# nh13/DWGSIM

Measured on AMD Instinct MI355X. Metric: M read-pairs/sec (2x150 bp PE), higher is better.
Workload: dtype u8

## Files before the change

dwgsim_amd/csrc/dw_common.hpp:

```cpp
#pragma once
#include <stdint.h>

#define DW_DEV __device__ __forceinline__
#include <dw_intrin.hpp>
#include <dw_probe.hpp>

namespace dw {

enum : uint32_t {
    D_WALK = 1,
    D_WALK_INSLEN = 2,
    D_WALK_INSBASE = 3,
    D_WALK_SITE = 7,
    D_WALK_SITE_REF = 26,
    D_PAIR = 4,
    D_PLACE = 5,
    D_PLACE_NORM = 6,
    D_BASE0 = 8,
    D_QUAL0 = 10,
    D_FLOW0 = 12,
    D_FLOW_REF = 32,
    D_FLOW_EV = 64,
    D_FLOW_PASS2 = 8,
    D_CALIB = 14,
// ... 51 lines not shown
{
    const U4 b = rng_block<UNIFORM_KEY>(k, dom, idx, att, 0, slot >> 1);
    return (slot & 1) ? u_hi(b) : u_lo(b);
}

DW_DEV uint64_t dbl_bits(double x) { union { double d; uint64_t u; } c; c.d = x; return c.u; }
DW_DEV double bits_dbl(uint64_t u) { union { double d; uint64_t u; } c; c.u = u; return c.d; }


template <bool NORMAL = false>
DW_DEV double det_log(double x)
{
    const double ln2_hi = 6.93147180369123816490e-01, ln2_lo = 1.90821492927058770002e-10,
                 Lg1 = 6.666666666666735130e-01, Lg2 = 3.999999999940941908e-01, Lg3 = 2.857142874366239149e-01,
                 Lg4 = 2.222219843214978396e-01, Lg5 = 1.818357216161805012e-01, Lg6 = 1.531383769920937332e-01,
                 Lg7 = 1.479819860511658591e-01;
    uint64_t b = dbl_bits(x);
    int32_t hx = (int32_t)(b >> 32), k = 0;
    if (!NORMAL && hx < 0x00100000) { x *= 0x1p54; k = -54; b = dbl_bits(x); hx = (int32_t)(b >> 32); }
    k += (hx >> 20) - 1023;
    hx &= 0x000fffff;
    int32_t i = (hx + 0x95f64) & 0x100000;
    x = bits_dbl(((uint64_t)(uint32_t)(hx | (i ^ 0x3ff00000)) << 32) | (b & 0xFFFFFFFFull));
    k += (i >> 20);
    const double f = x - 1.0, dk = (double)k;
    const double s = NORMAL ? div_mid(f, 2.0 + f) : f / (2.0 + f);
    const double z = s * s, w = z * z;
    const double t1 = w * (Lg2 + w * (Lg4 + w * Lg6));
    const double t2 = z * (Lg1 + w * (Lg3 + w * (Lg5 + w * Lg7)));
    const double R = t2 + t1;
    i = (hx - 0x6147a) | (0x6b851 - hx);
    if (i > 0) {
        const double hfsq = 0.5 * f * f;
        return dk * ln2_hi - ((hfsq - (s * (hfsq + R) + dk * ln2_lo)) - f);
    }
    return dk * ln2_hi - ((s * (f - R) - dk * ln2_lo) - f);
}

DW_DEV uint32_t geom_gap(uint32_t w, const uint32_t *lg, uint64_t R, int sR)
{
    const uint64_t X = ((uint64_t)w << 1) | 1ull;
    const int p = 63 - __clzll((long long)X);
    const uint64_t M = X << (63 - p);
    const uint32_t idx = (uint32_t)(M >> 55) & 0xFFu, r16 = (uint32_t)(M >> 39) & 0xFFFFu;
    const uint32_t t0 = lg[idx], t1 = lg[idx + 1];
    const uint32_t f = t0 + (uint32_t)(((uint64_t)(t1 - t0) * r16) >> 16);
    const uint64_t Lu = ((uint64_t)(33 - p) << 56) - ((uint64_t)f << 24);
    const uint64_t G = __umul64hi(Lu, R) >> sR;
    return G > 0x3FFFFFFFull ? 0x3FFFFFFFu : (uint32_t)G;
}

DW_DEV int lane_id() { return (int)(threadIdx.x & 63); }

DW_DEV uint32_t wave_incl_scan(uint32_t v)
{
#pragma unroll
    for (int d = 1; d < 64; d <<= 1) { uint32_t o = __shfl_up(v, d); if (lane_id() >= d) v += o; }
    return v;
}
DW_DEV uint64_t shfl_down_u64(uint64_t v, int d)
{
    uint32_t lo = __shfl_down((uint32_t)v, d), hi = __shfl_down((uint32_t)(v >> 32), d);
    return ((uint64_t)hi << 32) | lo;
}
DW_DEV uint64_t wave_sum_u64(uint64_t v)
{
#pragma unroll
    for (int d = 32; d >= 1; d >>= 1) v += shfl_down_u64(v, d);
    uint32_t lo = __shfl((uint32_t)v, 0), hi = __shfl((uint32_t)(v >> 32), 0);
    return ((uint64_t)hi << 32) | lo;
}
DW_DEV uint32_t wave_sum_u32(uint32_t v)
{
#pragma unroll
    for (int d = 32; d >= 1; d >>= 1) v += __shfl_down(v, d);
    return __shfl(v, 0);
}

constexpr uint64_t ST_AGG = 1ull << 62, ST_PREFIX = 2ull << 62, ST_VAL = (1ull << 62) - 1;

DW_DEV void status_store(uint64_t *p, uint64_t v) { __hip_atomic_store(p, v, __ATOMIC_RELAXED, __HIP_MEMORY_SCOPE_AGENT); }
DW_DEV uint64_t status_load(uint64_t *p) { return __hip_atomic_load(p, __ATOMIC_RELAXED, __HIP_MEMORY_SCOPE_AGENT); }

#ifndef DW_LB_SLEEP
#define DW_LB_SLEEP 2
#endif
#ifndef DW_LB_W
#define DW_LB_W 1
#endif
constexpr int LB_W = DW_LB_W;
DW_DEV uint64_t lookback_excl(uint64_t *status, uint32_t t, uint64_t aggregate, uint64_t base)
{
    const int lane = lane_id();
    if (t == 0) { if (lane == 0) status_store(&status[0], ST_PREFIX | ((base + aggregate) & ST_VAL)); return base; }
    if (lane == 0) status_store(&status[t], ST_AGG | (aggregate & ST_VAL));
    uint64_t excl = 0;
    int64_t k = (int64_t)t - 1;
    for (;;) {
        uint64_t v[LB_W];
#pragma unroll
        for (int w = 0; w < LB_W; ++w) {
            const int64_t idx = k - (int64_t)lane * LB_W - w;
            v[w] = idx >= 0 ? status_load(&status[idx]) : ST_PREFIX;
        }
#pragma unroll
        for (int w = 0; w < LB_W; ++w) {
            const int64_t idx = k - (int64_t)lane * LB_W - w;
            if (probe::off(2048) && (v[w] >> 62) == 0) v[w] = ST_PREFIX;
            while ((v[w] >> 62) == 0) { __builtin_amdgcn_s_sleep(DW_LB_SLEEP); v[w] = status_load(&status[idx]); }
        }
        uint64_t mine = 0; bool have = false;
#pragma unroll
        for (int w = 0; w < LB_W; ++w) { if (!have) mine += v[w] & ST_VAL; have = have || (v[w] >> 62) == 2; }
        const uint64_t pm = __ballot(have);
        const int first = pm ? (__ffsll((unsigned long long)pm) - 1) : 64;
        excl += wave_sum_u64(lane <= first ? mine : 0);
        if (pm) break;
        k -= 64 * LB_W;
    }
    if (lane == 0) status_store(&status[t], ST_PREFIX | ((excl + aggregate) & ST_VAL));
    return excl;
}

}
```

dwgsim_amd/csrc/dw_host.cpp:

```cpp
#include <hip/hip_runtime.h>
#include <math.h>
#include <stdio.h>
#include <stdlib.h>
#include <string.h>
#include <limits.h>
#include <ctype.h>
#include <stdarg.h>
#include <stdint.h>
#include <sys/mman.h>
#include <mutex>
#include <thread>
#include <string>
#include <vector>
#include <algorithm>
#include <array>
#include <stddef.h>
#include <type_traits>
#include "../../include/dwgsim_hip.h"
#include "dw_kernels.hpp"
#include "dw_launch.hpp"
#include "dw_mutin.hpp"
#include "dw_mem.hpp"

using namespace dw;
// ... 831 lines not shown

int dwgsim_hip_set_regions(dwgsim_hip_ctx_t *c, const char *path, const char *const *names, const int64_t *lens, int n_contigs, uint64_t *total_len)
{
    if (!c || !path || n_contigs < 0 || (n_contigs && (!names || !lens))) { if (c) c->err = "bad regions arguments"; return DWGSIM_HIP_ERR_ARG; }
    if (c->prm.amplicons) { c->err = "Error: cannot use a regions BED file (-x) when simulating amplicons (-a)\n"; return DWGSIM_HIP_ERR_ARG; }
    std::vector<ContigName> tab;
    for (int i = 0; i < n_contigs; ++i) tab.push_back(ContigName{names[i], lens[i]});
    std::string err;
    if (!parse_regions(path, tab, c->regions, err)) { c->err = err; c->has_regions = false; return DWGSIM_HIP_ERR_ARG; }
    c->has_regions = true;
    uint64_t tot = 0;
    for (size_t q = 0; q < c->regions.start.size(); ++q) tot += c->regions.end[q] - c->regions.start[q];
    if (total_len) *total_len = tot;
    return DWGSIM_HIP_OK;
}

int64_t dwgsim_hip_contig_region_length(dwgsim_hip_ctx_t *c, uint32_t contig_index, const uint8_t *ascii, int64_t len, int64_t *non_acgt, int64_t *region_bases)
{
    if (non_acgt) *non_acgt = 0;
    if (region_bases) *region_bases = len;
    if (!c || !c->has_regions) return len;
    int64_t m = 0, num_n = 0;
    for (size_t q = 0; q < c->regions.contig.size(); ++q) if (c->regions.contig[q] == contig_index) {
        m += c->regions.end[q] - c->regions.start[q];
        for (int64_t p = c->regions.start[q]; p <= (int64_t)c->regions.end[q]; ++p) { const int ch = (p >= 1 && p - 1 < len) ? ascii[p - 1] : 'N'; if (nt4(ch) >= 4) ++num_n; }
    }
    if (non_acgt) *non_acgt = num_n;
    if (region_bases) *region_bases = m;
    if (m == 0) return DWGSIM_HIP_SKIP_NO_REGION;
    if (0.95 < num_n / (double)m) return DWGSIM_HIP_SKIP_NON_ACGT;
    return m;
}

int dwgsim_hip_contig_set_placement_length(dwgsim_hip_ctx_t *c, int contig, int64_t l)
{
    int k = 0;
    Group *g = get_group(c, contig, &k);
    if (!g || l < 0) { if (c) c->err = "bad placement-length arguments"; return DWGSIM_HIP_ERR_ARG; }
    g->m[(size_t)k].l_place = l;
    return DWGSIM_HIP_OK;
}

int dwgsim_hip_set_mutation_input(dwgsim_hip_ctx_t *c, int type, const char *path, const char *const *names, const int64_t *lens, int n_contigs)
{
    if (!c || !path || type < 0 || type > 2 || n_contigs < 0 || (n_contigs && (!names || !lens))) { if (c) c->err = "bad mutation-input arguments"; return DWGSIM_HIP_ERR_ARG; }
    std::vector<ContigName> tab;
    for (int i = 0; i < n_contigs; ++i) tab.push_back(ContigName{names[i], lens[i]});
    std::string err;
    if (!parse_mutation_input(type, path, tab, c->mutin, err)) { c->err = err; c->has_mutin = false; return DWGSIM_HIP_ERR_ARG; }
    c->has_mutin = true;
    return DWGSIM_HIP_OK;
}

static int mut_debug_verdict(dwgsim_hip_ctx_t *c, const Group &g, uint64_t pre, uint64_t post)
{
    auto member_of = [&](uint64_t v) -> int { const int64_t p = (int64_t)(v >> 8); int k = 0; while (k + 1 < (int)g.m.size() && (int64_t)g.m[(size_t)k + 1].start <= p) ++k; return k; };
    uint64_t v = ~0ull;
    if (pre != ~0ull && post != ~0ull) v = member_of(post) < member_of(pre) ? post : pre;
    else v = pre != ~0ull ? pre : post;
    if (v == ~0ull) return DWGSIM_HIP_OK;
    static const char *what[4] = {"", "(c[0]&0x3) != (c[1]&0x3)", "(c[1]&0x3) != (c[2]&0x3)", "(c[0]&0x3) == (c[1]&0x3) || (c[0]&0x3) == (c[2]&0x3)"};
    const Member &m = g.m[(size_t)member_of(v)];
    char b[256]; snprintf(b, sizeof b, "dwgsim: src/mut.c: mut_debug: Assertion `%s' failed. [%s:%lld]\n", what[v & 3], m.name.c_str(), (long long)(v >> 8) - m.start + 1);
    c->err = b;
    return DWGSIM_HIP_ERR_FAILED;
}

static int ensure_ins(dwgsim_hip_ctx_t *c, Group &g, int h, size_t entries, size_t bases)
{
    GroupMem &M = g.mem;
    const size_t want = sizeof(int32_t) * (entries + entries / 4 + 64);
    for (DevMem *b : {&M.d_ins_pos[h], &M.d_ins_len[h], &M.d_ins_off[h]}) HIPC(c, reserve(c, *b, sizeof(int32_t) * entries, want));
    HIPC(c, reserve(c, M.d_ins_bases[h], bases + 16, bases + bases / 4 + 256 + 16));
    return DWGSIM_HIP_OK;
}

static void make_views(hipStream_t st, const Group &g)
{
    const GroupMem &M = g.mem;
    launch_make_view(st, M.d_cells[0].get(), M.d_cells[1].get(), (int64_t)padded_cells(g) & ~(int64_t)15, g.total, M.d_view[0].get(), M.d_view[1].get(),
                     M.d_summ[0].get<uint16_t>(), M.d_summ[1].get<uint16_t>(), M.d_summ2[0].get<uint16_t>(), M.d_summ2[1].get<uint16_t>());
}

static void dirty_chunks(hipStream_t st, bool restore, const Group &g)
{
    const GroupMem &M = g.mem;
    launch_dirty_chunks(st, restore, M.d_dirty.get<uint32_t>(), dirty_words(padded_cells(g)), g.total, M.d_ref.get(), M.d_refview.get(), M.d_refsumm.get<uint16_t>(), M.d_refsumm2.get<uint16_t>(),
                        M.d_cells[0].get(), M.d_cells[1].get(), M.d_view[0].get(), M.d_view[1].get(), M.d_summ[0].get<uint16_t>(), M.d_summ[1].get<uint16_t>(), M.d_summ2[0].get<uint16_t>(), M.d_summ2[1].get<uint16_t>());
}

static void justify(dwgsim_hip_ctx_t *c, hipStream_t st, const Event *ev, Count n, const ContigDev &cd)
{
    if (c->seq_justify) launch_justify_seq(st, ev, n, cd);
    else launch_justify(st, ev, n, cd, c->w_lo.get<int32_t>(), c->w_sufmin.get<int32_t>(), c->w_bound.get<uint8_t>());
}

static int64_t pack_walk_form(int attempt, bool file_driven, bool slots, int restore, bool dense)
{
    return (int64_t)attempt << 16 | (file_driven ? 1 : 0) << 12 | (slots ? 1 : 0) << 8 | restore << 4 | (dense ? 1 : 0);
}

static int walk_file_driven(dwgsim_hip_ctx_t *c, Group &g)
{
    hipStream_t st = c->walk_stream;
    const GroupMem &M = g.mem;
    WalkCounters *wc = c->d_wcounters.get<WalkCounters>();
    const uint32_t np = g.n_patch, nev = g.n_patch_ev;
    const size_t nev1 = nev ? nev : 1;
    if (np && (ensure(c, c->w_ppos, sizeof(int32_t) * np) || ensure(c, c->w_pcells, sizeof(uint16_t) * np) || ensure(c, c->w_ev, sizeof(Event) * nev1) ||
               ensure(c, c->w_lo, sizeof(int32_t) * nev1) || ensure(c, c->w_sufmin, sizeof(int32_t) * (nev1 + 64)) || ensure(c, c->w_bound, nev1))) return DWGSIM_HIP_ERR_DEVICE;
    c->walk_form = pack_walk_form(g.walk_attempt, true, false, g.walk_reset ? 2 : 0, true);
    HIPC(c, hipEventRecord(M.ev_walk0.get(), st));
    if (g.walk_reset) for (int h = 0; h < 2; ++h) if (const int rc = restore_pristine(c, g, h, R_CELLS, st)) return rc;
    HIPC(c, wc_fill(c, WC_FILE, 0xff, st));
    if (np) {
        HIPC(c, hipMemcpyAsync(c->w_ppos.get(), c->h_ppos.data(), sizeof(int32_t) * np, hipMemcpyHostToDevice, st));
        HIPC(c, hipMemcpyAsync(c->w_pcells.get(), c->h_pcells.data(), sizeof(uint16_t) * np, hipMemcpyHostToDevice, st));
        if (nev) HIPC(c, hipMemcpyAsync(c->w_ev.get(), c->h_pev.data(), sizeof(Event) * nev, hipMemcpyHostToDevice, st));
        launch_apply_patches(st, c->w_ppos.get<int32_t>(), c->w_pcells.get<uint16_t>(), np, M.d_cells[0].get(), M.d_cells[1].get());
        launch_mut_debug(st, M.d_ref.get(), M.d_cells[0].get(), M.d_cells[1].get(), g.total, &wc->mut_debug[0]);
        if (nev) justify(c, st, c->w_ev.get<Event>(), Count{nullptr, nev}, group_dev(g));
        launch_mut_debug(st, M.d_ref.get(), M.d_cells[0].get(), M.d_cells[1].get(), g.total, &wc->mut_debug[1]);
    }
    make_views(st, g);
    g.dirty_all = true;
    HIPC(c, hipGetLastError());
    HIPC(c, wc_fetch(c, M, WC_FILE, st));
    HIPC(c, hipEventRecord(M.ev_walk.get(), st));
    return DWGSIM_HIP_OK;
}

enum class Restore { None, Chunks, All };
struct WalkPlan {
    uint32_t cap; size_t ncap, cap_bases;
    uint32_t nblk;
    bool use_slots; uint32_t nbs, slot_cap; size_t slot_bytes;
    Restore restore;
    bool dense;
};

static WalkPlan walk_plan(const dwgsim_hip_ctx_t *c, const Group &g)
{
    WalkPlan P;
    P.cap = g.walk_cap; P.ncap = P.cap ? P.cap : 1; P.cap_bases = g.walk_cap_bases;
    P.nblk = (uint32_t)((g.total + SCAN_POS_PER_BLOCK - 1) / SCAN_POS_PER_BLOCK);
    P.nbs = site_scan_blocks(g.total);
    const double m = (double)site_scan_block_positions() * (c->prm.mut_rate > 0 ? c->prm.mut_rate : 0.0);
    P.slot_cap = (uint32_t)std::min<double>((double)site_scan_block_positions(), m + 8.0 * sqrt(m + 1.0) + 32.0);
    if (c->site_slot_cap >= 0) P.slot_cap = (uint32_t)std::max<int64_t>(1, c->site_slot_cap);
    P.slot_bytes = (size_t)P.nbs * P.slot_cap * sizeof(int32_t);
    P.use_slots = g.walk_attempt == 0 && c->site_slots != 0 && P.nbs > 0 && (c->site_slots > 0 || P.slot_bytes <= std::max<size_t>((size_t)64 << 20, P.ncap * 16));
    P.restore = g.walk_attempt > 0 || g.dirty_all ? Restore::All : g.dirty_any ? Restore::Chunks : Restore::None;
    P.dense = c->seq_justify || c->dense_view;
    return P;
}

static int walk_reserve(dwgsim_hip_ctx_t *c, Group &g, const WalkPlan &P)
{
    if (ensure(c, c->scratch_status, ((size_t)P.nblk + 2) * sizeof(uint64_t)) ||
        ensure(c, c->w_cand, sizeof(int32_t) * P.ncap) || ensure(c, c->w_ev, sizeof(Event) * P.ncap) ||
        ensure(c, c->w_flags, sizeof(uint4) * (P.ncap + 64)) ||
        ensure(c, c->w_lo, sizeof(int32_t) * P.ncap) || ensure(c, c->w_sufmin, sizeof(int32_t) * (P.ncap + 64)) ||
        ensure(c, c->w_bound, P.ncap)) return DWGSIM_HIP_ERR_DEVICE;
    for (int h = 0; h < 2; ++h) if (const int rc = ensure_ins(c, g, h, P.ncap, P.cap_bases)) return rc;
    if (P.use_slots && (ensure(c, c->w_slots, P.slot_bytes) || ensure(c, c->w_slot_aux, 2 * (size_t)P.nbs * sizeof(uint32_t)))) return DWGSIM_HIP_ERR_DEVICE;
    return DWGSIM_HIP_OK;
}

static int walk_launch(dwgsim_hip_ctx_t *c, Group &g, const WalkPlan &P)
{
    hipStream_t st = c->walk_stream;
    const WalkParams wp = walk_params(c);
    const SegTab seg = seg_tab(g);
    const GroupMem &M = g.mem;
    WalkCounters *wc = c->d_wcounters.get<WalkCounters>();
    int32_t *d_cand = c->w_cand.get<int32_t>(); Event *d_ev = c->w_ev.get<Event>(); uint4 *d_flags = c->w_flags.get<uint4>();
    uint32_t *tot4 = &wc->ins[0].entries;
    const Count nc{&wc->n_cand, P.cap};
    HIPC(c, wc_fill(c, WC_RANDOM, 0, st));
    if (P.use_slots) launch_site_scan_slots(st, M.d_refview.get(), g.total, seg, wp, c->w_slots.get<int32_t>(), P.slot_cap, c->w_slot_aux.get<uint32_t>(), d_cand, P.cap, &wc->n_cand, &wc->slot_over);
    else {
        uint64_t *d_status = c->scratch_status.get<uint64_t>();
        HIPC(c, hipMemsetAsync(d_status, 0, ((size_t)P.nblk + 2) * sizeof(uint64_t), st));
        launch_site_scan_list(st, M.d_refview.get(), g.total, seg, wp, d_status, d_status + P.nblk, d_cand, P.cap, &wc->n_cand);
    }
    launch_events(st, d_cand, nc, M.d_ref.get(), seg, wp, d_ev, &wc->max_del);
    launch_resolve(st, d_ev, nc, &wc->max_del, d_flags, tot4);
    ContigDev cd = group_dev(g);
    cd.tot4 = tot4; cd.cap_bases[0] = (uint32_t)std::min<size_t>(ins_bases_cap(g, 0), 0xFFFFFFFFu); cd.cap_bases[1] = (uint32_t)std::min<size_t>(ins_bases_cap(g, 1), 0xFFFFFFFFu);
    launch_apply(st, d_ev, nc, d_flags, cd, wp);
    justify(c, st, d_ev, nc, cd);
    if (P.dense) {
        make_views(st, g);
        g.dirty_all = true;
    } else {
        launch_mark_dirty(st, d_ev, nc, c->w_lo.get<int32_t>(), M.d_dirty.get<uint32_t>());
        dirty_chunks(st, false, g);
        g.dirty_any = true;
    }
    HIPC(c, hipGetLastError());
    return DWGSIM_HIP_OK;
}

static int walk_random(dwgsim_hip_ctx_t *c, Group &g)
{
    const WalkPlan P = walk_plan(c, g);
    if (const int rc = walk_reserve(c, g, P)) return rc;
    c->walk_form = pack_walk_form(g.walk_attempt, false, P.use_slots, (int)P.restore, P.dense);
    hipStream_t st = c->walk_stream;
    HIPC(c, hipEventRecord(g.mem.ev_walk0.get(), st));
    if (P.restore == Restore::All) { for (int h = 0; h < 2; ++h) if (const int rc = restore_pristine(c, g, h, R_ALL, st)) return rc; }
    else if (P.restore == Restore::Chunks) dirty_chunks(st, true, g);
    if (P.restore != Restore::None) { if (const int rc = clear_dirty(c, g, st)) return rc; g.dirty_all = g.dirty_any = false; }
    if (const int rc = walk_launch(c, g, P)) return rc;
    HIPC(c, wc_fetch(c, g.mem, WC_RANDOM, st));
    HIPC(c, hipEventRecord(g.mem.ev_walk.get(), st));
    return DWGSIM_HIP_OK;
}

static void collect_file_mutations(dwgsim_hip_ctx_t *c, const Group &g, HostIns (&hi)[2])
{
    c->h_ppos.clear(); c->h_pcells.clear(); c->h_pev.clear();
    for (size_t k = 0; k < g.m.size(); ++k) {
        const Member &m = g.m[k];
        for (size_t q = 0; q < m.rc.pos.size(); ++q) {
            c->h_ppos.push_back(m.rc.pos[q] + m.start); c->h_pcells.push_back(m.rc.cells[q]);
            if (m.rc.cells[q] & 0x3030) { Event e; e.pos = m.rc.pos[q] + m.start; e.type = 4; e.hap = 3; e.base = 0; e.live = 1; e.len = 1; e.seg = (uint32_t)k; c->h_pev.push_back(e); }
        }
        for (int h = 0; h < 2; ++h) for (const InsPayload &ip : m.rc.ins[h]) {
            hi[h].pos.push_back(ip.pos + m.start); hi[h].len.push_back((uint32_t)ip.bases.size()); hi[h].off.push_back((uint32_t)hi[h].bases.size());
            hi[h].bases.insert(hi[h].bases.end(), ip.bases.begin(), ip.bases.end());
        }
    }
}

static int upload_ins_tables(dwgsim_hip_ctx_t *c, Group &g, HostIns (&hi)[2])
{
    for (int h = 0; h < 2; ++h) {
        const size_t n = hi[h].pos.size(), nb = hi[h].bases.size();
        g.n_ins[h] = (uint32_t)n; g.n_ins_bases[h] = (uint32_t)nb;
        if (const int rc = ensure_ins(c, g, h, n ? n : 1, nb ? nb : 1)) return rc;
        if (n) for (const InsTable &t : ins_tables(g.mem, h, hi[h])) HIPC(c, hipMemcpy(t.dev, t.host, t.bytes, hipMemcpyHostToDevice));
    }
    return DWGSIM_HIP_OK;
}

static void initial_walk_caps(const dwgsim_hip_ctx_t *c, Group &g)
{
    double mean = 0;
    for (const Member &m : g.m) mean += (double)m.l * c->prm.mut_rate;
    g.walk_cap = (uint32_t)std::min<double>((double)g.total, mean + 8.0 * sqrt(mean + 1.0) + 256.0);
    g.walk_cap_bases = (size_t)g.walk_cap * 8 + 4096;
    if (c->walk_cap >= 0) { g.walk_cap = (uint32_t)c->walk_cap; g.walk_cap_bases = 1; }
}

int dwgsim_hip_mutate_async(dwgsim_hip_ctx_t *c, int contig)
{
    Group *gp = get_group(c, contig);
    if (!gp) return DWGSIM_HIP_ERR_ARG;
    Group &g = *gp;
    if (g.walk_pending) { c->err = "mutate: the group's previous walk was not waited for"; return DWGSIM_HIP_ERR_STATE; }
    for (const Slot &sl : c->slot) if (sl.pending && sl.group == c->handles[(size_t)contig].group) { c->err = "mutate: a batch that reads this group is still in flight (wait for it first)"; return DWGSIM_HIP_ERR_STATE; }
    HIPC(c, hipSetDevice(c->device));
    g.walk_reset = g.mutated;
    for (int h = 0; h < 2; ++h) g.n_ins[h] = g.n_ins_bases[h] = 0;
    g.mutated = true; g.n_cand = 0; g.list_valid = false;
    for (int h = 0; h < 2; ++h) g.hap_text[h].valid = false;
    g.walk_attempt = 0;
    if (g.total == 0) return DWGSIM_HIP_OK;
    if (c->has_mutin) {
        HIPC(c, hipStreamSynchronize(c->walk_stream));
        HostIns hi[2];
        collect_file_mutations(c, g, hi);
        g.n_patch = (uint32_t)c->h_ppos.size(); g.n_patch_ev = (uint32_t)c->h_pev.size();
        g.n_cand = g.n_patch_ev;
        HIPC(c, hipStreamSynchronize(c->walk_stream));
        if (const int rc = upload_ins_tables(c, g, hi)) return rc;
    } else initial_walk_caps(c, g);
    if (const int rc = c->has_mutin ? walk_file_driven(c, g) : walk_random(c, g)) return rc;
    g.walk_pending = true;
    return DWGSIM_HIP_OK;
}

static bool walk_fits(const WalkCounters &w, const Group &g)
{
    return !w.slot_over && w.n_cand <= g.walk_cap && w.ins[0].bases <= ins_bases_cap(g, 0) && w.ins[1].bases <= ins_bases_cap(g, 1);
}

static void exact_walk_caps(const WalkCounters &w, Group &g)
{
    g.walk_cap = (uint32_t)std::min<uint64_t>((uint64_t)g.total, (w.slot_over ? (uint64_t)w.n_cand_true : w.n_cand) + 16);
    g.walk_cap_bases = std::max<size_t>(g.walk_cap_bases, (size_t)std::max(w.ins[0].bases, w.ins[1].bases) * 2 + (size_t)g.walk_cap * 8 + 4096);
}

int dwgsim_hip_mutate_wait(dwgsim_hip_ctx_t *c, int contig)
{
// ... 495 lines not shown
    if (per_range) for (int q = 0; q < n; ++q) per_range[q] = 0;
    Launch L;
    if (const int rc = build_ranges(c, r, n, PLACE_PAIRS, L)) return rc;
    const uint64_t n_pairs = L.n_pairs; const uint32_t n_blocks = L.nblk;
    if (n_pairs == 0) return DWGSIM_HIP_OK;
    Group &g = *L.g;
    HIPC(c, hipSetDevice(c->device));
    hipStream_t st = c->count_stream;
    if (g.walk_pending) { if (const int rc = dwgsim_hip_mutate_wait(c, g.first_handle)) return rc; }
    if (g.mem.ev_walk.get() && g.mutated) HIPC(c, hipStreamWaitEvent(st, g.mem.ev_walk.get(), 0));
    if (const int rc = sim_form(c, L.f)) return rc;
    SimArgs &a = L.a; fill_sim_args(c, g, L.f, a);
    const size_t ns = L.segs.size();
    if (ensure(c, c->place_rand, sizeof(uint32_t) * ((size_t)n_blocks + 1)) || ensure(c, c->place_segs, sizeof(SimSeg) * ns) ||
        ensure(c, c->place_aux, PLACE_LISTS * 16 * sizeof(uint32_t) + sizeof(uint64_t) * ns)) return DWGSIM_HIP_ERR_DEVICE;
    if (sizeof(SimSeg) * ns > c->h_place_segs.cap() || sizeof(uint64_t) * ns > c->h_range_rand.cap()) HIPC(c, hipStreamSynchronize(st));
    HIPC(c, c->h_place_segs.reserve(sizeof(SimSeg) * ns, sizeof(SimSeg) * (ns + 64))); HIPC(c, c->h_range_rand.reserve(sizeof(uint64_t) * ns, sizeof(uint64_t) * (ns + 64)));
    const uint64_t *h_range_rand = c->h_range_rand.get<uint64_t>();
    memcpy(c->h_place_segs.get(), L.segs.data(), sizeof(SimSeg) * ns);
    HIPC(c, hipMemcpyAsync(c->place_segs.get(), c->h_place_segs.get(), sizeof(SimSeg) * ns, hipMemcpyHostToDevice, st));
    a.segs = c->place_segs.get<SimSeg>(); a.n_seg = (int32_t)ns; a.n_blocks = n_blocks; a.n_pairs = n_pairs;
    a.block_rand = c->place_rand.get<uint32_t>(); a.counters = c->pcounters.dev();
    const uint64_t waves = (uint64_t)n_blocks * (PLACE_PAIRS / 64);
    const uint32_t cap_full = (uint32_t)((waves + PLACE_LISTS - 1) / PLACE_LISTS) * 64u;
    uint32_t cap = (uint32_t)std::min<uint64_t>(cap_full, 1024 + n_pairs / PLACE_LISTS / 8);
    if (c->place_cap >= 0 && (uint64_t)c->place_cap < cap) cap = (uint32_t)c->place_cap;
    for (int attempt = 0;; ++attempt) {
        if (ensure(c, c->place_list, sizeof(uint32_t) * (size_t)cap * PLACE_LISTS)) return DWGSIM_HIP_ERR_DEVICE;
        a.place_list = c->place_list.get<uint32_t>(); a.place_list_cap = cap;
        a.place_list_n = c->place_aux.get<uint32_t>(); a.range_rand = reinterpret_cast<uint64_t *>(c->place_aux.get<uint8_t>() + PLACE_LISTS * 16 * sizeof(uint32_t));
        HIPC(c, hipMemsetAsync(c->pcounters.dev(), 0, N_COUNTERS * sizeof(uint64_t), st));
        HIPC(c, hipMemsetAsync(c->place_aux.get(), 0, PLACE_LISTS * 16 * sizeof(uint32_t) + sizeof(uint64_t) * ns, st));
        HIPC(c, hipEventRecord(c->ev_cnt0, st));
        launch_place(st, a);
        HIPC(c, hipEventRecord(c->ev_cnt1, st));
        HIPC(c, hipGetLastError());
        HIPC(c, hipMemcpyAsync(c->pcounters.host(), c->pcounters.dev(), N_COUNTERS * sizeof(uint64_t), hipMemcpyDeviceToHost, st));
        HIPC(c, hipMemcpyAsync(c->h_range_rand.get(), a.range_rand, sizeof(uint64_t) * ns, hipMemcpyDeviceToHost, st));
        HIPC(c, hipStreamSynchronize(st));
        { float ms = 0; if (hipEventElapsedTime(&ms, c->ev_cnt0, c->ev_cnt1) == hipSuccess) c->count_us += 1e3 * ms; else (void)hipGetLastError(); }
        if (!(c->pcounters.host()[2] & 16) || attempt > 0) break;
        cap = cap_full;
    }
    if (c->pcounters.host()[2] & 16) { c->err = "count_random: the list of undecided pairs overflowed twice"; return DWGSIM_HIP_ERR_FAILED; }
    if (c->pcounters.host()[2]) { char b[128]; snprintf(b, sizeof b, "\r[dwgsim_core] failed to generate a read after %d trials\n", MAX_ATTEMPTS + 1); c->err = b; return DWGSIM_HIP_ERR_FAILED; }
    c->place_open = c->pcounters.host()[5];
    uint64_t total = 0;
    for (int q = 0, si = 0; q < n; ++q) if (r[q].n_pairs) { total += h_range_rand[si]; if (per_range) per_range[q] = h_range_rand[si]; ++si; }
    if (n_random) *n_random = total;
    return DWGSIM_HIP_OK;
}

int dwgsim_hip_count_random(dwgsim_hip_ctx_t *c, int contig, uint64_t first_ii, uint64_t n_pairs, uint64_t *n_random)
{
    dwgsim_hip_range_t r; memset(&r, 0, sizeof r); r.contig = contig; r.first_ii = first_ii; r.n_pairs = n_pairs;
    return dwgsim_hip_count_random_ranges(c, &r, 1, n_random, nullptr);
}

int dwgsim_hip_set_fail_carry(dwgsim_hip_ctx_t *c, uint64_t carry)
{
    if (!c) return DWGSIM_HIP_ERR_ARG;
    c->carry_override = carry; c->has_carry_override = true;
    return DWGSIM_HIP_OK;
}

static SimPlan sim_plan(const dwgsim_hip_ctx_t *c, const Launch &L)
{
    const dwgsim_hip_params_t &p = c->prm; const SimForm &f = L.f;
    const uint64_t n_pairs = L.n_pairs; const size_t nblk = L.nblk;
    SimPlan P{};
    const int fixed_max = std::max(L.fixed_max, c->rand_fixed_len);
    for (int j = 0; j < 2; ++j) if (p.length[j] > 0) P.cap[j] = (size_t)n_pairs * (size_t)(1 + fixed_max + 120 + 3 + 2 * (p.data_type == 2 ? f.cap : p.length[j]) + 4);
    int bw_bytes = 0, bw_pairs = 0;
    while (bw_bytes < 63 && (((uint64_t)P.cap[0] | 1ull) >> bw_bytes)) ++bw_bytes;
    while (bw_pairs < 63 && (n_pairs >> bw_pairs)) ++bw_pairs;
    P.lb_shift = bw_bytes; P.too_many = p.data_type != 2 && bw_bytes + bw_pairs > 62;
    P.cap[2] = P.cap[0] + P.cap[1];
    if (!L.a.p.has_bwa) P.cap[0] = P.cap[1] = 0;
    if (!L.a.p.has_bfast) P.cap[2] = 0;
    P.block_rand = sizeof(uint32_t) * nblk;
    if (!f.split) P.status = 4 * sizeof(uint64_t) * nblk;
    else { P.split_state = sizeof(uint32_t) * (size_t)f.lds_words * SIM_THREADS * nblk; P.split_hand = 16 * (size_t)SIM_THREADS * nblk; P.split_agg = 16 * nblk; P.split_pre = 32 * nblk; P.split_chunk = 32 * (nblk / 1024 + 1); }
    P.meta = sizeof(uint32_t) * ((size_t)n_pairs + 8);
    P.fail_summ = ((size_t)((n_pairs + 256ull * 64 - 1) / (256ull * 64)) * 4 + 2) * sizeof(uint64_t);
    P.scratch = f.dt == 2 || (f.dt < 2 && f.nthr == SIM_THREADS_LONG);
    if (P.scratch) {
        const int cu_per_xcd = (c->n_cu >= 64 && c->n_cu % 8 == 0) ? c->n_cu / 8 : c->n_cu;
        const bool ion = p.data_type == 2;
        const int per_cu = sim_blocks_per_cu(f.lds, ion ? 8 : 32);
        P.flow_slots = c->flow_slots > 0 ? c->flow_slots : cu_per_xcd * per_cu;
        if ((uint64_t)P.flow_slots > (uint64_t)nblk) P.flow_slots = (int32_t)nblk;
        if (ion) {
            const size_t slot_bytes = (size_t)flow_words_per_lane(f.lds_words) * (size_t)SIM_THREADS * sizeof(uint32_t);
            const size_t fit = std::max<size_t>(1, ((size_t)4 << 30) / (slot_bytes * 8));
            if ((size_t)P.flow_slots > fit) P.flow_slots = (int32_t)fit;
        }
        const size_t words = (ion ? (size_t)flow_words_per_lane(f.lds_words) * (size_t)SIM_THREADS : (size_t)f.lds_words * (size_t)SIM_THREADS_LONG) * (size_t)P.flow_slots * 8;
        P.flow_scratch = words * sizeof(uint32_t); P.flow_free = sizeof(uint64_t) * (256 + 8 * nblk);
    }
    P.segs = sizeof(SimSeg) * L.segs.size();
    if (c->gzip_on) {
        size_t chunks = 0;
        for (int t = 0; t < 3; ++t) { P.gz_chunks[t] = (size_t)gz_chunks(P.cap[t]); chunks += P.gz_chunks[t]; if (P.cap[t]) P.gz_cap[t] = (size_t)gz_capacity(P.cap[t]); }
        P.gz_status = sizeof(uint64_t) * (chunks ? chunks : 1);
    }
    return P;
}

static int sim_reserve(dwgsim_hip_ctx_t *c, int slot, const SimPlan &P)
{
    Slot &sl = c->slot[slot]; DevMem *out = c->out[slot];
    if (sl.fetch_in_flight) { HIPC(c, hipStreamWaitEvent(c->stream, sl.ev_fetched, 0)); bool grows = false; for (int t = 0; t < 3; ++t) if (P.cap[t] + 64 > out[t].cap()) grows = true; if (grows) HIPC(c, hipEventSynchronize(sl.ev_fetched)); sl.fetch_in_flight = false; }
    for (int t = 0; t < 3; ++t) if (ensure(c, out[t], P.cap[t] + 64)) return DWGSIM_HIP_ERR_DEVICE;
    if (ensure(c, c->block_rand, P.block_rand) || ensure(c, c->status_all, P.status) ||
        ensure(c, c->split_state, P.split_state) || ensure(c, c->split_hand, P.split_hand) || ensure(c, c->split_agg, P.split_agg) || ensure(c, c->split_pre, P.split_pre) || ensure(c, c->split_chunk, P.split_chunk) ||
        ensure(c, c->meta, P.meta) || ensure(c, c->fail_summ, P.fail_summ) || ensure(c, c->flow_scratch, P.flow_scratch) || ensure(c, c->flow_free, P.flow_free) || ensure(c, sl.segs, P.segs)) return DWGSIM_HIP_ERR_DEVICE;
    HIPC(c, sl.h_segs.reserve(P.segs, P.segs + 64 * sizeof(SimSeg)));
    for (int t = 0; t < 3; ++t) if (P.gz_cap[t] && ensure(c, sl.gz_out[t], P.gz_cap[t] + 64)) return DWGSIM_HIP_ERR_DEVICE;
    return ensure(c, sl.gz_status, P.gz_status);
}

static ChainSet sim_chain(dwgsim_hip_ctx_t *c, Slot &sl, const dwgsim_hip_range_t *r, int n, bool set_rand, bool rerun)
{
    if (rerun) return ChainSet{sl.d_rerun_chain.get<uint64_t>(), 1, 1, 0};
    const dwgsim_hip_range_t *r_first = nullptr, *r_last = nullptr;
    for (int q = 0; q < n; ++q) if (r[q].n_pairs) { if (!r_first) r_first = &r[q]; r_last = &r[q]; }
    if (!r_first) { r_first = &r[0]; r_last = &r[n - 1]; }
    const bool continues = c->chain_contig == r_first->contig && c->chain_next_ii == r_first->first_ii && r_first->first_ii != 0;
    const ChainSet ch{c->d_chain.get<uint64_t>(), set_rand ? 1 : 0, (c->has_carry_override || !continues) ? 1 : 0, c->has_carry_override ? c->carry_override : 0};
    c->has_carry_override = false; c->chain_contig = r_last->contig; c->chain_next_ii = r_last->first_ii + r_last->n_pairs;
    if (sl.ranges.data() != r) sl.ranges.assign(r, r + n);
    return ch;
}

static int sim_launch(dwgsim_hip_ctx_t *c, int slot, Launch &L, const SimPlan &P, const ChainSet &ch, uint64_t rand_base, bool rerun)
{
    Slot &sl = c->slot[slot]; SimArgs &a = L.a; const SimForm &f = L.f;
    const uint64_t n_pairs = L.n_pairs; const uint32_t nblk = L.nblk;
    for (int t = 0; t < 3; ++t) sl.out_bytes[t] = sl.gz_bytes[t] = 0;
    sl.n_pairs = n_pairs; sl.empty = n_pairs == 0;
    if (n_pairs == 0) { if (ch.set_rand || ch.set_carry) launch_chain_set(c->stream, ch.words, rand_base, ch.set_rand, ch.carry, ch.set_carry); return DWGSIM_HIP_OK; }
    uint32_t opens = 0; for (const SimSeg &s : L.segs) opens |= s.contig_start;
    memcpy(sl.h_segs.get(), L.segs.data(), P.segs);
    HIPC(c, hipMemcpyAsync(sl.segs.get(), sl.h_segs.get(), P.segs, hipMemcpyHostToDevice, c->stream));
    a.segs = sl.segs.get<SimSeg>(); a.n_seg = (int32_t)L.segs.size(); a.n_blocks = nblk; a.n_pairs = n_pairs; a.chain = ch.words; a.lb_shift = P.lb_shift;
    a.meta = c->meta.get<uint32_t>(); a.block_rand = c->block_rand.get<uint32_t>(); a.counters = sl.counters.dev();
    for (int t = 0; t < 3; ++t) a.out[t] = c->out[slot][t].get<uint8_t>();
    for (int j = 0; j < 4; ++j) a.status[j] = f.split ? nullptr : c->status_all.get<uint64_t>() + (size_t)j * (size_t)nblk;
    if (f.split) { a.split_state = c->split_state.get<uint32_t>(); a.split_hand = c->split_hand.get<uint32_t>(); a.split_agg = c->split_agg.get<uint32_t>(); a.split_pre = c->split_pre.get<uint64_t>(); a.split_chunk = c->split_chunk.get<uint64_t>(); }
    if (P.scratch) { a.flow_scratch = c->flow_scratch.get<uint32_t>(); a.flow_free = c->flow_free.get<uint64_t>(); a.flow_slots = P.flow_slots; }
    sl.group = c->handles[(size_t)L.g->first_handle].group;
    launch_init(c->stream, sl.counters.dev(), (uint32_t)N_COUNTERS, a.status[0], f.split ? 0 : 4 * (uint64_t)nblk, a.flow_free, a.flow_free ? 256 + 8 * (uint64_t)nblk : 0,
                ch.words, rand_base, ch.set_rand, ch.carry, ch.set_carry);
    HIPC(c, hipEventRecord(sl.ev_k0, c->stream));
    c->sim_form = (int64_t)f.nthr << 20 | f.lpp << 16 | f.out << 12 | f.dt << 8 | f.wr << 4 | f.split;
    if (!launch_simulate(c->stream, a, f)) { c->err = "simulate: no k_simulate instance for this form"; return DWGSIM_HIP_ERR_FAILED; }
    HIPC(c, hipEventRecord(sl.ev_k1, c->stream));
    sl.cap_mult = c->flow_cap_mult;
    if (!rerun) launch_failrule(c->stream, a.meta, n_pairs, opens, c->fail_summ.get<uint64_t>(), sl.counters.dev(), c->d_chain.get<uint64_t>());
    if (c->gzip_on) {
        HIPC(c, hipMemsetAsync(sl.gz_status.get(), 0, P.gz_status, c->stream));
        size_t off = 0;
        for (int t = 0; t < 3; ++t) {
            if (P.cap[t] == 0) continue;
            launch_gzip(c->stream, a.out[t], &sl.counters.dev()[4 + t], P.cap[t], sl.gz_out[t].get<uint8_t>(), P.gz_cap[t], sl.gz_status.get<uint64_t>() + off, &sl.counters.dev()[28 + t], &sl.counters.dev()[24 + t], &sl.counters.dev()[2],
                        c->d_crc_table.get<uint32_t>(), c->d_crc_shift.get<uint32_t>());
            off += P.gz_chunks[t];
        }
    }
    HIPC(c, hipEventRecord(sl.ev_end, c->stream));
    HIPC(c, hipGetLastError());
    HIPC(c, hipMemcpyAsync(sl.counters.host(), sl.counters.dev(), N_COUNTERS * sizeof(uint64_t), hipMemcpyDeviceToHost, c->stream));
    HIPC(c, hipEventRecord(sl.ev_done, c->stream));
    sl.pending = true;
    return DWGSIM_HIP_OK;
}

static int sim_enqueue(dwgsim_hip_ctx_t *c, const dwgsim_hip_range_t *r, int n, uint64_t rand_base, int slot, bool rerun)
{
    if (!c || slot < 0 || slot >= DWGSIM_HIP_SLOTS) { if (c) c->err = "bad simulate arguments"; return DWGSIM_HIP_ERR_ARG; }
    if (c->slot[slot].pending) { c->err = "simulate: the slot still holds a batch that was not waited for"; return DWGSIM_HIP_ERR_STATE; }
    Launch L;
    if (const int rc = sim_resolve(c, r, n, L)) return rc;
    HIPC(c, hipSetDevice(c->device));
    const SimPlan P = sim_plan(c, L);
    if (P.too_many) { c->err = "too many pairs in one call"; return DWGSIM_HIP_ERR_ARG; }
    if (L.n_pairs) { if (const int rc = sim_reserve(c, slot, P)) return rc; }
    return sim_launch(c, slot, L, P, sim_chain(c, c->slot[slot], r, n, rand_base != DWGSIM_HIP_RAND_CHAIN, rerun), rand_base, rerun);
}

int dwgsim_hip_simulate_ranges_async(dwgsim_hip_ctx_t *c, const dwgsim_hip_range_t *r, int n, uint64_t rand_base, int slot) { return sim_enqueue(c, r, n, rand_base, slot, false); }

int dwgsim_hip_simulate_async(dwgsim_hip_ctx_t *c, int contig, uint64_t first_ii, uint64_t n_pairs, uint64_t rand_base, int slot)
{
    dwgsim_hip_range_t r; memset(&r, 0, sizeof r); r.contig = contig; r.first_ii = first_ii; r.n_pairs = n_pairs;
    return dwgsim_hip_simulate_ranges_async(c, &r, 1, rand_base, slot);
}

int dwgsim_hip_wait(dwgsim_hip_ctx_t *c, int slot, dwgsim_hip_batch_t *out)
{
    if (!c || slot < 0 || slot >= DWGSIM_HIP_SLOTS) { if (c) c->err = "bad slot"; return DWGSIM_HIP_ERR_ARG; }
    Slot &sl = c->slot[slot];
    if (out) memset(out, 0, sizeof *out);
    if (sl.empty) { sl.pending = false; return DWGSIM_HIP_OK; }
    if (!sl.pending) { c->err = "wait: no batch was enqueued on this slot"; return DWGSIM_HIP_ERR_STATE; }
    HIPC(c, hipSetDevice(c->device));
    HIPC(c, hipEventSynchronize(sl.ev_done));
    sl.pending = false;
    uint64_t *h = sl.counters.host();
    if ((h[2] & 2) && !(h[2] & ~(2ull | 8ull)) && c->prm.data_type == 2) {
        uint64_t keep[8]; for (int q = 0; q < 6; ++q) keep[q] = h[16 + q];
        const uint64_t base = h[22];
        while (h[2] & 2) {
            if (sl.cap_mult >= c->flow_cap_mult) {
                if ((int64_t)flow_base_capacity(c) * (int64_t)c->flow_cap_mult * 2 > (int64_t)FLOW_CAP_MAX) break;
                c->flow_cap_mult *= 2;
            }
            if (const int rc = sim_enqueue(c, sl.ranges.data(), (int)sl.ranges.size(), base, slot, true)) return rc;
            HIPC(c, hipEventSynchronize(sl.ev_done));
            sl.pending = false;
        }
        for (int q = 0; q < 6; ++q) h[16 + q] = keep[q];
    }
    if (h[2] & 4) { c->err = "dwgsim-hip: no fragment placement satisfied the target regions (-x) after 2^20 tries (the reference would not terminate)\n"; return DWGSIM_HIP_ERR_FAILED; }
    if (h[2] & 2) { c->err = "dwgsim-hip: a read outgrew its buffer (or degenerated) in the flow-error model\n"; return DWGSIM_HIP_ERR_FAILED; }
    if ((h[2] & ~8ull) || h[20]) {
        char b[128]; snprintf(b, sizeof b, "\r[dwgsim_core] failed to generate a read after %d trials\n", MAX_ATTEMPTS + 1); c->err = b; return DWGSIM_HIP_ERR_FAILED;
    }
    if (h[2] & 8) { c->err = "dwgsim-hip: the gzip output buffer is too small for this text\n"; return DWGSIM_HIP_ERR_FAILED; }
    for (int t = 0; t < 3; ++t) { sl.out_bytes[t] = h[4 + t]; sl.gz_bytes[t] = h[24 + t]; }
    if (c->phases) {
        uint64_t tot = 0; for (int k = 0; k < 8; ++k) tot += h[8 + k];
        fprintf(stderr, "[phases]");
        for (int k = 0; k < 8; ++k) fprintf(stderr, " p%d=%.1f%%", k, tot ? 100.0 * h[8 + k] / tot : 0.0);
        fprintf(stderr, " (ticks %llu)\n", (unsigned long long)tot);
    }
// ... 220 lines not shown
```

dwgsim_amd/csrc/dw_launch.hpp:

```cpp
#pragma once
#include <hip/hip_runtime.h>
#include "dw_kernels.hpp"

namespace dw {
void launch_pack(hipStream_t st, const uint8_t *ascii, uint8_t *ref, uint8_t *h0, uint8_t *h1, int64_t l);
void launch_site_scan_list(hipStream_t st, const uint8_t *refview, int64_t l, SegTab seg, WalkParams wp, uint64_t *status, uint64_t *ticket, int32_t *out, uint32_t cap, uint64_t *n_out);
uint32_t site_scan_blocks(int64_t l);
uint32_t site_scan_block_positions();
void launch_site_scan_slots(hipStream_t st, const uint8_t *refview, int64_t l, SegTab seg, WalkParams wp, int32_t *slots, uint32_t slot_cap, uint32_t *aux, int32_t *out, uint32_t cap, uint64_t *n_out, uint32_t *over);
void launch_mark_dirty(hipStream_t st, const Event *ev, Count n, const int32_t *lo, uint32_t *dirty);
void launch_dirty_chunks(hipStream_t st, bool restore, const uint32_t *dirty, uint32_t n_words, int64_t l_live, const uint8_t *ref, const uint8_t *refview, const uint16_t *refsumm, const uint16_t *refsumm2,
                         uint8_t *cells0, uint8_t *cells1, uint8_t *view0, uint8_t *view1, uint16_t *summ0, uint16_t *summ1, uint16_t *summ2_0, uint16_t *summ2_1);
void launch_scan_excl(hipStream_t st, uint32_t *data, uint32_t n, uint64_t *total_out);
void launch_compact(hipStream_t st, const uint16_t *mask, const uint32_t *block_base, int32_t *out, int64_t l, uint32_t cap);
void launch_events(hipStream_t st, const int32_t *cand, Count n, const uint8_t *ref, SegTab seg, WalkParams wp, Event *ev, uint32_t *max_del);
void walk_debug_seg_min(uint32_t rows);
void launch_resolve(hipStream_t st, Event *ev, Count n, const uint32_t *max_del, uint4 *flags, uint32_t *tot4);
void launch_apply(hipStream_t st, Event *ev, Count n, const uint4 *flags, ContigDev c, WalkParams wp);
void launch_justify_seq(hipStream_t st, const Event *ev, Count n, ContigDev c);
void launch_justify(hipStream_t st, const Event *ev, Count n, ContigDev c, int32_t *lo, int32_t *sufmin, uint8_t *bound);
void launch_mut_debug(hipStream_t st, const uint8_t *ref, const uint8_t *h0, const uint8_t *h1, int64_t l, uint64_t *verdict);
void launch_make_view(hipStream_t st, const uint8_t *cells0, const uint8_t *cells1, int64_t n_cells, int64_t l_live, uint8_t *view0, uint8_t *view1, uint16_t *summ0, uint16_t *summ1, uint16_t *summ2_0, uint16_t *summ2_1);
void launch_apply_patches(hipStream_t st, const int32_t *pos, const uint16_t *cells, uint32_t n, uint8_t *h0, uint8_t *h1);
void launch_collect_mask(hipStream_t st, const uint8_t *h0, const uint8_t *h1, int64_t l, uint16_t *mask, uint32_t *block_count);
void launch_gather(hipStream_t st, const int32_t *pos, uint32_t n, const uint8_t *ref, const uint8_t *h0, const uint8_t *h1, uint32_t *cells);
void launch_hap_len(hipStream_t st, HapDev h, SegTab seg, int64_t l, uint32_t *block_count);
void launch_hap_write(hipStream_t st, HapDev h, SegTab seg, int64_t l, const uint32_t *block_base, const HapRec *rec, uint32_t n_rec, const uint8_t *pool, uint32_t width, uint8_t *text);
void launch_place(hipStream_t st, const SimArgs &a);
bool launch_simulate(hipStream_t st, const SimArgs &a, const SimForm &f);
void launch_calibrate(hipStream_t st, const CalibArgs &a);
void launch_failrule(hipStream_t st, const uint32_t *meta, uint64_t n_pairs, uint32_t opens_contig, uint64_t *summ, uint64_t *counters, uint64_t *chain);
void launch_chain_set(hipStream_t st, uint64_t *chain, uint64_t rand_base, int set_rand, uint64_t carry, int set_carry);
void launch_init(hipStream_t st, uint64_t *counters, uint32_t n_counters, uint64_t *z0, uint64_t n0, uint64_t *z1, uint64_t n1, uint64_t *chain, uint64_t rand_base, int set_rand, uint64_t carry, int set_carry);
void launch_selftest_lazy(hipStream_t st, int mode, uint32_t first, uint64_t n, double sigma, float qk, float qeps, float qlmin, int qnear1, uint64_t *out);
uint64_t gz_chunks(uint64_t n);
uint64_t gz_capacity(uint64_t n);
void gz_host_tables(uint32_t *crc_table, uint32_t *crc_shift);
void launch_gzip(hipStream_t st, const uint8_t *text, const uint64_t *n_dev, uint64_t text_cap, uint8_t *out, uint64_t out_cap, uint64_t *status, uint64_t *ticket, uint64_t *total, uint64_t *flags,
                 const uint32_t *crc_table, const uint32_t *crc_shift);
void launch_count_byte(hipStream_t st, const uint8_t *text, uint64_t n, uint32_t byte, uint64_t *out);
void launch_selftest_fp64(hipStream_t st, uint32_t seed, uint64_t n, uint64_t *mism);
void launch_selftest_text(hipStream_t st, uint64_t first, uint64_t n, uint64_t stride, uint64_t *out);
void launch_selftest_gap(hipStream_t st, const uint32_t *lg, uint64_t R, int sR, uint32_t first, uint64_t n, uint32_t g_lo, uint32_t g_cnt, uint32_t *chg, uint64_t *out);
}
```

dwgsim_amd/csrc/dw_simulate.hip:

```cpp
#include <algorithm>
#include "dw_read.hpp"
#include "dw_launch.hpp"

#ifndef DW_PART
#define DW_PART -1
#endif
#define DW_HAS(part) (DW_PART == -1 || DW_PART == (part))
#ifndef DW_SIM_WAVES
#define DW_SIM_WAVES 5
#endif
#ifndef DW_SOLID_WAVES
#define DW_SOLID_WAVES 4
#endif
#ifndef DW_SIM_WAVES_BOTH
#define DW_SIM_WAVES_BOTH 4
#endif
#ifndef DW_SIMB_WAVES
#define DW_SIMB_WAVES 6
#endif
#ifndef DW_IONA_WAVES
#define DW_IONA_WAVES 4
#endif
#ifndef DW_IONL_WAVES
#define DW_IONL_WAVES 3
// ... 900 lines not shown
        }
        done += (uint32_t)(i1 - i0);
    }
    const uint32_t s0 = wave_sum_u32(up), s1 = wave_sum_u32(clip), s2 = wave_sum_u32(done);
    if ((threadIdx.x & 63) == 0) {
        if (s0) atomicAdd((unsigned long long *)&out[0], (unsigned long long)s0);
        if (s1) atomicAdd((unsigned long long *)&out[1], (unsigned long long)s1);
        atomicAdd((unsigned long long *)&out[2], (unsigned long long)s2);
    }
}
void launch_selftest_gap(hipStream_t st, const uint32_t *lg, uint64_t R, int sR, uint32_t first, uint64_t n, uint32_t g_lo, uint32_t g_cnt, uint32_t *chg, uint64_t *out)
{
    const uint64_t nb = cdiv(cdiv(n, GAP_RUN), 256);
    hipLaunchKernelGGL(k_selftest_gap, dim3((uint32_t)(nb < (1u << 16) ? (nb ? nb : 1) : (1u << 16))), dim3(256), 0, st, lg, R, sR, first, n, g_lo, g_cnt, chg, out);
}
void launch_selftest_fp64(hipStream_t st, uint32_t seed, uint64_t n, uint64_t *mism)
{
    hipLaunchKernelGGL(k_selftest_fp64, dim3(cdiv(n, 256)), dim3(256), 0, st, seed, n, mism);
}
__global__ void __launch_bounds__(1024) k_split_scan1(SimArgs a)
{
    __shared__ uint32_t sm[3][16];
    const uint32_t t = blockIdx.x * 1024u + threadIdx.x;
    uint4 g = make_uint4(0, 0, 0, 0);
    if (t < a.n_blocks) g = reinterpret_cast<const uint4 *>(a.split_agg)[t];
    const uint32_t v[3] = {g.x, g.y, g.z};
    uint32_t ex[3], tot[3];
    block_excl_scan_n<3>(v, sm, ex, tot);
    if (t < a.n_blocks) { uint64_t *o = a.split_pre + 4 * (size_t)t; o[0] = ex[0]; o[1] = ex[1]; o[2] = ex[2]; }
    if (threadIdx.x == 0) { uint64_t *c = a.split_chunk + 4 * (size_t)blockIdx.x; c[0] = tot[0]; c[1] = tot[1]; c[2] = tot[2]; }
}
__global__ void __launch_bounds__(64) k_split_scan2(SimArgs a, int lpp)
{
    const uint32_t nch = (a.n_blocks + 1023u) / 1024u;
    uint64_t run[3] = {0, 0, 0};
    for (uint32_t base = 0; base < nch; base += 64u) {
        const uint32_t c = base + threadIdx.x;
        uint64_t v[3] = {0, 0, 0};
        if (c < nch) for (int k = 0; k < 3; ++k) v[k] = a.split_chunk[4 * (size_t)c + k];
        uint64_t inc[3];
#pragma unroll
        for (int k = 0; k < 3; ++k) {
            uint64_t x = v[k];
#pragma unroll
            for (int d = 1; d < 64; d <<= 1) { const uint32_t ol = (uint32_t)__shfl_up((int)(uint32_t)x, d), oh = (uint32_t)__shfl_up((int)(uint32_t)(x >> 32), d); if (lane_id() >= d) x += ((uint64_t)oh << 32) | ol; }
            inc[k] = x;
        }
        if (c < nch) for (int k = 0; k < 3; ++k) a.split_chunk[4 * (size_t)c + k] = run[k] + inc[k] - v[k];
        for (int k = 0; k < 3; ++k) { const uint32_t lo = (uint32_t)__shfl((int)(uint32_t)inc[k], 63), hi = (uint32_t)__shfl((int)(uint32_t)(inc[k] >> 32), 63); run[k] += ((uint64_t)hi << 32) | lo; }
    }
    if (threadIdx.x == 0) {
        const uint64_t H = hex_digits_sum(a.chain[0], run[0]), G1 = run[1] + H, G2 = run[2] + (lpp == 2 ? H : 0ull);
        const uint64_t nreads = a.n_pairs * (uint64_t)((a.p.len[1] > 0) ? 2 : 1);
        a.counters[3] = run[0];
        a.counters[4] = a.p.has_bwa ? G1 : 0;
        a.counters[5] = a.p.has_bwa ? G2 : 0;
        a.counters[6] = !a.p.has_bfast ? 0 : G1 + G2 - 2 * nreads;
    }
}

struct FailSeg { uint64_t P, S; uint32_t R, bad; };
DW_DEV FailSeg failseg_join(const FailSeg &a, const FailSeg &b)
{
    FailSeg r;
    r.bad = a.bad | b.bad | ((a.R && a.S + b.P > (uint64_t)MAX_ATTEMPTS) ? 1u : 0u);
    r.P = a.R ? a.P : a.P + b.P;
    r.S = b.R ? b.S : a.S + b.S;
    r.R = a.R | b.R;
    return r;
}
DW_DEV FailSeg failseg_wave_join(FailSeg x, int cnt)
{
    const int lane = lane_id();
#pragma unroll
    for (int d = 1; d < 64; d <<= 1) {
        FailSeg o;
        o.P = ((uint64_t)(uint32_t)__shfl_down((int)(uint32_t)(x.P >> 32), d) << 32) | (uint32_t)__shfl_down((int)(uint32_t)x.P, d);
        o.S = ((uint64_t)(uint32_t)__shfl_down((int)(uint32_t)(x.S >> 32), d) << 32) | (uint32_t)__shfl_down((int)(uint32_t)x.S, d);
        o.R = (uint32_t)__shfl_down((int)x.R, d); o.bad = (uint32_t)__shfl_down((int)x.bad, d);
        if ((lane & (2 * d - 1)) == 0 && lane + d < cnt) x = failseg_join(x, o);
    }
    return x;
}
constexpr int FAIL_PAIRS_PER_THREAD = 64;
__global__ void __launch_bounds__(256) k_failrule_a(const uint32_t *__restrict__ meta, uint64_t n_pairs, const uint64_t *__restrict__ counters, uint64_t *__restrict__ summ)
{
    __shared__ FailSeg seg[4];
    if (counters[1] == 0) return;
    const uint64_t first = ((uint64_t)blockIdx.x * 256 + threadIdx.x) * FAIL_PAIRS_PER_THREAD;
    FailSeg s{0, 0, 0, 0};
    for (int q4 = 0; q4 < FAIL_PAIRS_PER_THREAD && first + q4 < n_pairs; q4 += 4) {
        const uint4 v = *reinterpret_cast<const uint4 *>(meta + first + q4);
        const uint32_t mm[4] = {v.x, v.y, v.z, v.w};
#pragma unroll
        for (int u = 0; u < 4; ++u) {
            if (first + q4 + u >= n_pairs) break;
            const uint32_t m = mm[u];
            if (m & 0x40000000u) s = failseg_join(s, FailSeg{0, 0, 1, 0});
            FailSeg one{m & 0x3fffffffu, 0, (m >> 31) ? 0u : 1u, 0};
            if (!one.R) one.S = one.P;
            s = failseg_join(s, one);
        }
    }
    s = failseg_wave_join(s, 64);
    if ((threadIdx.x & 63) == 0) seg[threadIdx.x >> 6] = s;
    __syncthreads();
    if (threadIdx.x == 0) {
        FailSeg t = seg[0];
        for (int k = 1; k < 4; ++k) t = failseg_join(t, seg[k]);
        summ[4 * (uint64_t)blockIdx.x + 0] = t.P; summ[4 * (uint64_t)blockIdx.x + 1] = t.S;
        summ[4 * (uint64_t)blockIdx.x + 2] = t.R; summ[4 * (uint64_t)blockIdx.x + 3] = t.bad;
    }
}
__global__ void __launch_bounds__(64) k_failrule_b(const uint64_t *__restrict__ summ, uint32_t n_blocks, uint64_t n_pairs, uint32_t opens_contig, uint64_t *__restrict__ counters, uint64_t *__restrict__ chain)
{
    FailSeg t{0, 0, (counters[3] < n_pairs || opens_contig) ? 1u : 0u, 0};
    if (counters[1] != 0) {
        const uint32_t per = (n_blocks + 63) / 64, b0 = threadIdx.x * per, b1 = b0 + per < n_blocks ? b0 + per : n_blocks;
        FailSeg x{0, 0, 0, 0};
        for (uint32_t b = b0; b < b1; ++b) {
            const FailSeg nx{summ[4 * (uint64_t)b], summ[4 * (uint64_t)b + 1], (uint32_t)summ[4 * (uint64_t)b + 2], (uint32_t)summ[4 * (uint64_t)b + 3]};
            x = (b == b0) ? nx : failseg_join(x, nx);
        }
        t = failseg_wave_join(x, per ? (int)((n_blocks + per - 1) / per) : 0);
    }
    if (threadIdx.x == 0) {
        const uint64_t carry = chain[1];
        const FailSeg all = failseg_join(FailSeg{carry, carry, 0, 0}, t);
        counters[16] = t.P; counters[17] = t.S; counters[18] = t.R; counters[19] = t.bad;
        counters[20] = (all.bad || all.P > (uint64_t)MAX_ATTEMPTS || all.S > (uint64_t)MAX_ATTEMPTS) ? 1 : 0;
        counters[21] = all.S;
        chain[1] = all.S;
        counters[22] = chain[0];
        chain[0] += counters[3];
    }
}
void launch_failrule(hipStream_t st, const uint32_t *meta, uint64_t n_pairs, uint32_t opens_contig, uint64_t *summ, uint64_t *counters, uint64_t *chain)
{
    const uint32_t nb = cdiv(n_pairs, 256ull * FAIL_PAIRS_PER_THREAD);
    hipLaunchKernelGGL(k_failrule_a, dim3(nb), dim3(256), 0, st, meta, n_pairs, counters, summ);
    hipLaunchKernelGGL(k_failrule_b, dim3(1), dim3(64), 0, st, summ, nb, n_pairs, opens_contig, counters, chain);
}
__global__ void __launch_bounds__(64) k_chain_set(uint64_t *chain, uint64_t rand_base, int set_rand, uint64_t carry, int set_carry)
{
    if (threadIdx.x != 0) return;
    if (set_rand) chain[0] = rand_base;
    if (set_carry) chain[1] = carry;
}
void launch_chain_set(hipStream_t st, uint64_t *chain, uint64_t rand_base, int set_rand, uint64_t carry, int set_carry)
{
    hipLaunchKernelGGL(k_chain_set, dim3(1), dim3(64), 0, st, chain, rand_base, set_rand, carry, set_carry);
}
__global__ void __launch_bounds__(256) k_launch_init(uint64_t *counters, uint32_t n_counters, uint64_t *z0, uint64_t n0, uint64_t *z1, uint64_t n1, uint64_t *chain, uint64_t rand_base, int set_rand, uint64_t carry, int set_carry)
{
    const uint64_t i = (uint64_t)blockIdx.x * 256 + threadIdx.x, stride = (uint64_t)gridDim.x * 256;
    if (i < n_counters) counters[i] = 0;
    for (uint64_t k = i; k < n0; k += stride) z0[k] = 0;
    for (uint64_t k = i; k < n1; k += stride) z1[k] = 0;
    if (i == 0) { if (set_rand) chain[0] = rand_base; if (set_carry) chain[1] = carry; }
}
void launch_init(hipStream_t st, uint64_t *counters, uint32_t n_counters, uint64_t *z0, uint64_t n0, uint64_t *z1, uint64_t n1, uint64_t *chain, uint64_t rand_base, int set_rand, uint64_t carry, int set_carry)
{
    const uint64_t most = n0 > n1 ? n0 : n1, want = (most + 255) / 256;
    hipLaunchKernelGGL(k_launch_init, dim3((uint32_t)(want < 1 ? 1 : want > 2048 ? 2048 : want)), dim3(256), 0, st, counters, n_counters, z0, n0, z1, n1, chain, rand_base, set_rand, carry, set_carry);
}
__global__ void __launch_bounds__(256) k_count_byte(const uint8_t *__restrict__ text, uint64_t n, uint32_t byte, uint64_t *out)
{
    const uint32_t pat = byte * 0x01010101u;
    uint32_t cnt = 0;
    const uint64_t nvec = n / 16;
    for (uint64_t v = (uint64_t)blockIdx.x * 256 + threadIdx.x; v < nvec; v += (uint64_t)gridDim.x * 256) {
        const uint4 q = reinterpret_cast<const uint4 *>(text)[v];
        const uint32_t w[4] = {q.x ^ pat, q.y ^ pat, q.z ^ pat, q.w ^ pat};
#pragma unroll
        for (int k = 0; k < 4; ++k) cnt += (uint32_t)__popc(~(((w[k] & 0x7F7F7F7Fu) + 0x7F7F7F7Fu) | w[k] | 0x7F7F7F7Fu));
    }
    if (blockIdx.x == 0 && threadIdx.x == 0) for (uint64_t q = nvec * 16; q < n; ++q) cnt += text[q] == byte;
    const uint32_t s = wave_sum_u32(cnt);
    if ((threadIdx.x & 63) == 0 && s) atomicAdd((unsigned long long *)out, (unsigned long long)s);
}
void launch_count_byte(hipStream_t st, const uint8_t *text, uint64_t n, uint32_t byte, uint64_t *out)
{
    hipLaunchKernelGGL(k_count_byte, dim3(4096), dim3(256), 0, st, text, n, byte, out);
}
void launch_place(hipStream_t st, const SimArgs &a)
{
    hipLaunchKernelGGL(k_place, dim3(a.n_blocks), dim3(PLACE_PAIRS), 0, st, a);
    const uint32_t per_list = (uint32_t)std::min<uint64_t>(16, std::max<uint64_t>(1, ((uint64_t)a.place_list_cap + 1023) / 1024));
    hipLaunchKernelGGL(k_place_rest, dim3(PLACE_LISTS * per_list), dim3(128), 0, st, a);
    launch_scan_excl(st, a.block_rand, a.n_blocks, &a.counters[3]);
    hipLaunchKernelGGL(k_range_counts, dim3(cdiv((uint64_t)a.n_seg, 256)), dim3(256), 0, st, a);
}
void launch_split_scan(hipStream_t st, const SimArgs &a, int lpp)
{
    hipLaunchKernelGGL(k_split_scan1, dim3(cdiv(a.n_blocks, 1024)), dim3(1024), 0, st, a);
    hipLaunchKernelGGL(k_split_scan2, dim3(1), dim3(64), 0, st, a, lpp);
}
#endif

#if DW_HAS(4)
__global__ void __launch_bounds__(PAIRS_PER_BLOCK) k_calibrate(CalibArgs a)
{
    DW_DYN_SHARED(uint32_t, dyn_lds);
    __shared__ FlowTables s_ft;
    const int tid = (int)threadIdx.x, nthr = PAIRS_PER_BLOCK;
    if (tid < 64) s_ft.flow[tid] = a.flow[tid];
    __syncthreads();
    fill_flow_tables(s_ft, a.flow_len, tid, nthr, a.flow);
    __syncthreads();
    const uint64_t jj = a.first_read + (uint64_t)blockIdx.x * PAIRS_PER_BLOCK + (uint64_t)tid;
    uint32_t *buf = a.scratch + (size_t)blockIdx.x * ((size_t)a.lds_words * nthr) + tid;
    const int capb = 16 * a.lds_words;
    int32_t n_err = 0; int s_out = 0;
    const bool live = jj < a.n_reads;
    const RngKey key{a.seed, 0u};
    const uint32_t dom = D_CALIB + (uint32_t)a.end;
    if (live) {
        const int h0 = ((capb - a.len) & ~7) >> 3;
        for (int w = 0; w * 8 < a.len; ++w) {
            const U4 q0 = rng_block(key, dom, jj, 0, 0, (uint32_t)(2 * w)), q1 = rng_block(key, dom, jj, 0, 0, (uint32_t)(2 * w + 1));
            const uint32_t rw[8] = {q0.x, q0.y, q0.z, q0.w, q1.x, q1.y, q1.z, q1.w};
            uint32_t pairs = 0;
#pragma unroll
            for (int b = 0; b < 8; ++b) if (w * 8 + b < a.len) pairs |= (rw[b] >> 30) << (2 * b);
            const int h = h0 + w;
            reinterpret_cast<uint16_t *>(buf + (h >> 1) * nthr)[h & 1] = (uint16_t)pairs;
        }
    }
    {
        FlowRng rg; rg.seed = a.seed; rg.contig = 0; rg.dom = dom; rg.att = 1; rg.evt = 0; rg.s = 0; rg.ii = jj; rg.w0 = rg.w1 = rg.w2 = rg.w3 = 0;
        const int so = flow_errors(live, rg, s_ft, a.flow_len, a.thr, a.gap_r, a.gap_s, buf, dyn_lds + tid, nthr, 2 * a.stack_words, a.len, 0, capb, &n_err);
        if (live) { s_out = so; if (s_out < 0) { atomicOr((unsigned long long *)&a.counters[2], 2ull); s_out = 0; n_err = 0; } }
    }
    const uint32_t es = wave_sum_u32((uint32_t)n_err), ls = wave_sum_u32((uint32_t)s_out);
    if ((tid & 63) == 0) { atomicAdd((unsigned long long *)&a.counters[8], (unsigned long long)es); atomicAdd((unsigned long long *)&a.counters[9], (unsigned long long)ls); }
}
void launch_calibrate(hipStream_t st, const CalibArgs &a)
{
    hipLaunchKernelGGL(k_calibrate, dim3(cdiv(std::min(a.chunk_reads, a.n_reads - a.first_read), (uint64_t)PAIRS_PER_BLOCK)), dim3(PAIRS_PER_BLOCK), (size_t)a.stack_words * PAIRS_PER_BLOCK * 4, st, a);
}
#endif

#define DW_SIM_OUTS(X, LPP, DT, NTHR, WR, SPLIT) X(LPP, 1, DT, NTHR, WR, SPLIT) X(LPP, 2, DT, NTHR, WR, SPLIT) X(LPP, 3, DT, NTHR, WR, SPLIT)
#define DW_SIM_PART_1(X)  DW_SIM_OUTS(X, 2, 0, 256, 0, 0) DW_SIM_OUTS(X, 2, 0, 256, 1, 0)
#define DW_SIM_PART_2(X)  DW_SIM_OUTS(X, 1, 0, 256, 0, 0) DW_SIM_OUTS(X, 1, 0, 256, 1, 0)
#define DW_SIM_PART_3(X)  DW_SIM_OUTS(X, 2, 2, 256, 1, 0)
#define DW_SIM_PART_4(X)  DW_SIM_OUTS(X, 1, 2, 256, 1, 0)
// ... 58 lines not shown
```

dwgsim_amd/csrc/dw_walk.hip:

```cpp
#include "dw_device.hpp"
#include "dw_launch.hpp"
#include <stdlib.h>

namespace dw {

__global__ void k_pack(const uint8_t *__restrict__ ascii, uint8_t *__restrict__ ref, uint8_t *__restrict__ h0,
                       uint8_t *__restrict__ h1, int64_t l)
{
    const int64_t nchunk = (l + 15) >> 4;
    for (int64_t ch = (int64_t)blockIdx.x * blockDim.x + threadIdx.x; ch < nchunk; ch += (int64_t)gridDim.x * blockDim.x) {
        const int64_t p0 = ch << 4;
        uint32_t w[4] = {0, 0, 0, 0};
        if (p0 + 16 <= l) {
            const uint4 v = *reinterpret_cast<const uint4 *>(ascii + p0);
            const uint32_t in[4] = {v.x, v.y, v.z, v.w};
#pragma unroll
            for (int q = 0; q < 4; ++q)
#pragma unroll
                for (int b = 0; b < 4; ++b) w[q] |= code_of_ascii((in[q] >> (8 * b)) & 0xff) << (8 * b);
        } else {
            for (int b = 0; b < 16; ++b) { const uint32_t c = (p0 + b < l) ? code_of_ascii(ascii[p0 + b]) : 4u; w[b >> 2] |= c << (8 * (b & 3)); }
        }
        const uint4 o = make_uint4(w[0], w[1], w[2], w[3]);
        *reinterpret_cast<uint4 *>(ref + p0) = o;
// ... 7 lines not shown
struct SiteChain {
    uint32_t m, w0, w1, w2, w3;
    DW_DEV uint32_t gap(RngKey key, uint32_t q, const WalkParams &wp, const uint32_t *lg)
    {
        if ((m & 3u) == 0u) { const U4 b = rng_block<false>(key, D_WALK_SITE, (uint64_t)q, 0, 0, m >> 2); w0 = b.x; w1 = b.y; w2 = b.z; w3 = b.w; }
        const uint32_t k = m & 3u; ++m;
        const uint32_t w = (k & 2u) ? ((k & 1u) ? w3 : w2) : ((k & 1u) ? w1 : w0);
        return wp.mut_thr >= 0x100000000ull ? 0u : geom_gap(w, lg, wp.gap_r, wp.gap_s);
    }
};
template <class F>
DW_DEV uint32_t site_window(const uint8_t *__restrict__ refview, int64_t l_total, const SegTab &seg, const WalkParams &wp, const uint32_t *lg, int64_t g0, F &&f)
{
    if (g0 >= l_total || wp.mut_thr == 0) return 0;
    const uint32_t sk = seg_of(seg, g0);
    const int64_t p0 = g0 - seg.start[sk], l = seg.len[sk];
    if (p0 >= l) return 0;
    const RngKey key{wp.seed, seg.cindex[sk]};
    const uint32_t q = (uint32_t)(p0 >> 8);
    const uint32_t lim = l - p0 < SITE_WINDOW ? (uint32_t)(l - p0) : (uint32_t)SITE_WINDOW;
    SiteChain ch; ch.m = 0; ch.w0 = ch.w1 = ch.w2 = ch.w3 = 0;
    uint32_t n = 0;
    for (uint32_t S = ch.gap(key, q, wp, lg); S < lim; S += 1u + ch.gap(key, q, wp, lg)) {
        const int64_t g = g0 + S;
        const uint32_t nib = (refview[g >> 1] >> (4 * (g & 1))) & 15u;
        if (nib < 4u) { f(g, n); ++n; }
    }
    return n;
}

__global__ void __launch_bounds__(SITE_THREADS) k_site_scan_list(const uint8_t *__restrict__ refview, int64_t l_total, SegTab seg, WalkParams wp, uint64_t *status, uint64_t *ticket,
                                                              int32_t *__restrict__ out, uint32_t cap, uint64_t *n_out, uint32_t n_blocks)
{
    __shared__ uint32_t sm[1][16], s_lg[FLOW_LG_ENTRIES];
    __shared__ uint32_t s_t; __shared__ uint64_t s_base;
    for (int q = (int)threadIdx.x; q < FLOW_LG_ENTRIES; q += SITE_THREADS) s_lg[q] = wp.lg[q];
    if (threadIdx.x == 0) s_t = (uint32_t)atomicAdd((unsigned long long *)ticket, 1ull);
    __syncthreads();
    const uint32_t t = uniform_u32(s_t);
    const int64_t g0 = ((int64_t)t * SITE_THREADS + threadIdx.x) * SITE_WINDOW;
    const uint32_t cnt[1] = {site_window(refview, l_total, seg, wp, s_lg, g0, [](int64_t, uint32_t) {})};
    uint32_t off[1], tot[1];
    block_excl_scan_n<1>(cnt, sm, off, tot);
    if (threadIdx.x < 64) {
        const uint64_t g = lookback_excl(status, t, tot[0], 0);
        if (threadIdx.x == 0) { s_base = g; if (t + 1 == n_blocks) *n_out = g + tot[0]; }
    }
    __syncthreads();
    const uint64_t at0 = s_base + off[0];
    if (cnt[0]) (void)site_window(refview, l_total, seg, wp, s_lg, g0, [&](int64_t g, uint32_t k) { if (at0 + k < cap) out[at0 + k] = (int32_t)g; });
}

__global__ void __launch_bounds__(SITE_THREADS) k_site_scan_slots(const uint8_t *__restrict__ refview, int64_t l_total, SegTab seg, WalkParams wp, int32_t *__restrict__ slots, uint32_t slot_cap,
                                                               uint32_t *__restrict__ slot_cnt)
{
    __shared__ uint32_t sm[1][16], s_lg[FLOW_LG_ENTRIES];
    for (int q = (int)threadIdx.x; q < FLOW_LG_ENTRIES; q += SITE_THREADS) s_lg[q] = wp.lg[q];
    __syncthreads();
    const uint32_t t = blockIdx.x;
    const int64_t g0 = ((int64_t)t * SITE_THREADS + threadIdx.x) * SITE_WINDOW;
    const uint32_t cnt[1] = {site_window(refview, l_total, seg, wp, s_lg, g0, [](int64_t, uint32_t) {})};
    uint32_t off[1], tot[1];
    block_excl_scan_n<1>(cnt, sm, off, tot);
    if (threadIdx.x == 0) slot_cnt[t] = tot[0];
    int32_t *const slot = slots + (size_t)t * slot_cap;
    const uint32_t at0 = off[0];
    if (cnt[0]) (void)site_window(refview, l_total, seg, wp, s_lg, g0, [&](int64_t g, uint32_t k) { if (at0 + k < slot_cap) slot[at0 + k] = (int32_t)g; });
}
__global__ void __launch_bounds__(1024) k_slot_scan(const uint32_t *__restrict__ slot_cnt, uint32_t nb, uint32_t slot_cap, uint32_t *__restrict__ slot_base, uint64_t *n_out, uint32_t *over)
{
    __shared__ uint32_t sm[17];
    __shared__ uint32_t s_over;
    if (threadIdx.x == 0) s_over = 0;
    const uint32_t per = (nb + 1023u) / 1024u, a = threadIdx.x * per, b = a + per < nb ? a + per : nb;
    uint32_t sum = 0; bool big = false;
    for (uint32_t q = a; q < b; ++q) { const uint32_t c = slot_cnt[q]; sum += c; big |= c > slot_cap; }
    uint32_t total;
    uint32_t run = block_excl_scan(sum, sm, &total);
    if (big) atomicOr(&s_over, 1u);
    for (uint32_t q = a; q < b; ++q) { slot_base[q] = run; run += slot_cnt[q]; }
    __syncthreads();
    if (threadIdx.x == 0) { const bool o = s_over != 0; *n_out = o ? 0ull : (uint64_t)total; if (o) { over[0] = 1u; over[1] = total; } }
}
__global__ void __launch_bounds__(256) k_slot_gather(const int32_t *__restrict__ slots, uint32_t slot_cap, const uint32_t *__restrict__ slot_cnt, const uint32_t *__restrict__ slot_base,
                                                     int32_t *__restrict__ out, uint32_t cap)
{
    const uint32_t t = blockIdx.x, base = slot_base[t];
    uint32_t n = slot_cnt[t]; if (n > slot_cap) n = slot_cap;
    for (uint32_t k = threadIdx.x; k < n; k += 256u) if (base + k < cap) out[base + k] = slots[(size_t)t * slot_cap + k];
}

__global__ void k_mark_dirty(const Event *__restrict__ ev, Count nc, const int32_t *__restrict__ lo, uint32_t *__restrict__ dirty)
{
    const uint32_t n = count_of(nc), k = blockIdx.x * blockDim.x + threadIdx.x;
    if (k >= n) return;
    const Event e = ev[k];
    if (!e.live) return;
    const int64_t right = (int64_t)e.pos + (e.type == 2 ? (int64_t)e.len - 1 : 0);
    const int64_t a = (int64_t)(lo[k] < e.pos ? lo[k] : e.pos) >> 6, b = right >> 6;
    for (int64_t q = a; q <= b; ++q) atomicOr(&dirty[q >> 5], 1u << (q & 31));
}
template <bool RESTORE, bool PER_CHUNK>
__global__ void __launch_bounds__(256) k_dirty_chunks(const uint32_t *__restrict__ dirty, uint32_t n_words, int64_t l_live, const uint8_t *__restrict__ ref, const uint8_t *__restrict__ refview,
                                                      const uint16_t *__restrict__ refsumm, const uint16_t *__restrict__ refsumm2,
                                                      uint8_t *__restrict__ cells0, uint8_t *__restrict__ cells1, uint8_t *__restrict__ view0, uint8_t *__restrict__ view1,
                                                      uint16_t *__restrict__ summ0, uint16_t *__restrict__ summ1, uint16_t *__restrict__ summ2_0, uint16_t *__restrict__ summ2_1)
{
    const uint64_t gid = (uint64_t)blockIdx.x * 256u + threadIdx.x;
    const uint32_t w = PER_CHUNK ? (uint32_t)(gid >> 5) : (uint32_t)gid;
    const bool in = w < n_words;
    const uint32_t touched = in ? dirty[w] : 0u;
    if (PER_CHUNK) { if (!__ballot(touched != 0u)) return; }
    else if (!touched) return;
    uint32_t bits = PER_CHUNK ? ((touched >> (gid & 31u)) & 1u) << (gid & 31u) : touched;
    uint32_t fine[2] = {0u, 0u};
    const bool mine = bits != 0u;
    while (bits) {
        const int q = __ffs((int)bits) - 1; bits &= bits - 1;
        const int64_t ch = (int64_t)w * 32 + q, first = ch * SUMM_CELLS;
        if (RESTORE) {
#pragma unroll
            for (int k = 0; k < SUMM_CELLS / 16; ++k) { const uint4 v = *reinterpret_cast<const uint4 *>(ref + first + 16 * k); *reinterpret_cast<uint4 *>(cells0 + first + 16 * k) = v; *reinterpret_cast<uint4 *>(cells1 + first + 16 * k) = v; }
#pragma unroll
            for (int k = 0; k < SUMM_CELLS / 32; ++k) { const uint4 v = *reinterpret_cast<const uint4 *>(refview + (first >> 1) + 16 * k); *reinterpret_cast<uint4 *>(view0 + (first >> 1) + 16 * k) = v; *reinterpret_cast<uint4 *>(view1 + (first >> 1) + 16 * k) = v; }
            const uint16_t sv = refsumm[ch]; summ0[ch] = sv; summ1[ch] = sv;
        } else {
#pragma unroll
            for (int h = 0; h < 2; ++h) {
                const uint8_t *cells = h ? cells1 : cells0; uint8_t *view = h ? view1 : view0;
                uint32_t indel = 0, non_acgt = 0;
#pragma unroll
                for (int half = 0; half < SUMM_CELLS / 32; ++half) {
                    uint32_t out[4] = {0, 0, 0, 0};
#pragma unroll
                    for (int qq = 0; qq < 2; ++qq) {
                        const int64_t at = first + 32 * half + 16 * qq;
                        const uint4 v = *reinterpret_cast<const uint4 *>(cells + at);
                        const uint32_t wd[4] = {v.x, v.y, v.z, v.w};
#pragma unroll
                        for (int b = 0; b < 16; ++b) {
                            const uint32_t c = (wd[b >> 2] >> (8 * (b & 3))) & 0xffu, ty = c & TMASK, base = c & 0xfu;
                            const uint32_t nib = ty == T_NONE ? (base < 4 ? base : base == 4 ? 8u : 9u) : (ty == T_SUB && base < 4) ? 4u + base : 15u;
                            const int cell = 16 * qq + b;
                            out[cell >> 3] |= nib << (4 * (cell & 7));
                        }
#pragma unroll
                        for (int k = 0; k < 4; ++k) {
                            const int64_t rem = l_live - (at + 4 * k);
                            const uint32_t lm = rem >= 4 ? 0xFFFFFFFFu : rem <= 0 ? 0u : ((1u << (8 * (int)rem)) - 1u);
                            indel += (uint32_t)__popc(wd[k] & lm & 0x10101010u);
                            non_acgt |= wd[k] & lm & 0x0C0C0C0Cu;
                        }
                    }
                    *reinterpret_cast<uint4 *>(view + ((first + 32 * half) >> 1)) = make_uint4(out[0], out[1], out[2], out[3]);
                }
                fine[h] = indel | (non_acgt ? 0x8000u : 0u);
                (h ? summ1 : summ0)[ch] = (uint16_t)fine[h];
            }
        }
    }
    static_assert(SUMM2_CELLS / SUMM_CELLS == 16, "a coarse summary = the sixteen lanes of half a bitmap word");
    if (!PER_CHUNK) {
#pragma unroll
        for (int half = 0; half < 2; ++half) {
            if (!((touched >> (16 * half)) & 0xFFFFu)) continue;
            const int64_t s2 = (int64_t)w * 2 + half;
            if (s2 * SUMM2_CELLS >= l_live) continue;
            if (RESTORE) { const uint16_t sv = refsumm2[s2]; summ2_0[s2] = sv; summ2_1[s2] = sv; }
            else {
#pragma unroll
                for (int h = 0; h < 2; ++h) {
                    const uint16_t *sm1 = h ? summ1 : summ0;
                    uint32_t cnt = 0, fl = 0;
                    for (int k = 0; k < SUMM2_CELLS / SUMM_CELLS; ++k) { const int64_t c2 = s2 * (SUMM2_CELLS / SUMM_CELLS) + k; if (c2 * SUMM_CELLS < l_live) { const uint32_t v = sm1[c2]; cnt += v & 0x7fffu; fl |= v & 0x8000u; } }
                    (h ? summ2_1 : summ2_0)[s2] = (uint16_t)(cnt | fl);
                }
            }
        }
        return;
    }
    const int q = (int)(gid & 31u);
    const int64_t ch = (int64_t)w * 32 + q;
    const int64_t s2 = (int64_t)w * 2 + (q >> 4);
    const bool live2 = in && ((touched >> (16 * (q >> 4))) & 0xFFFFu) != 0u && s2 * SUMM2_CELLS < l_live;
    if (RESTORE) { if (live2 && (q & 15) == 0) { const uint16_t sv = refsumm2[s2]; summ2_0[s2] = sv; summ2_1[s2] = sv; } }
    else {
#pragma unroll
        for (int h = 0; h < 2; ++h) {
            uint32_t v = 0;
            if (live2 && ch * SUMM_CELLS < l_live) v = mine ? fine[h] : (uint32_t)(h ? summ1 : summ0)[ch];
            uint32_t cnt = v & 0x7fffu, fl = v & 0x8000u;
#pragma unroll
            for (int m = 1; m < 16; m <<= 1) { cnt += (uint32_t)__shfl_xor((int)cnt, m); fl |= (uint32_t)__shfl_xor((int)fl, m); }
            if (live2 && (q & 15) == 0) (h ? summ2_1 : summ2_0)[s2] = (uint16_t)(cnt | fl);
        }
    }
}

__global__ void k_scan_excl(uint32_t *data, uint32_t n, uint64_t *total_out)
{
    __shared__ uint32_t sm[2][1][16];
    uint64_t grand = 0; int buf = 0;
    for (uint32_t base = 0; base < n; base += blockDim.x, buf ^= 1) {
        const uint32_t i = base + threadIdx.x;
        const uint32_t v[1] = {i < n ? data[i] : 0u};
        uint32_t ex[1], total[1];
        block_excl_scan_n<1>(v, sm[buf], ex, total);
        if (i < n) data[i] = ex[0] + (uint32_t)grand;
        grand += total[0];
    }
    if (total_out && threadIdx.x == 0) *total_out = grand;
}

__global__ void k_compact(const uint16_t *__restrict__ mask, const uint32_t *__restrict__ block_base, int32_t *__restrict__ out, uint32_t cap)
{
    __shared__ uint32_t sm[17];
    uint32_t bits = mask[(int64_t)blockIdx.x * SCAN_THREADS + threadIdx.x];
    uint32_t total;
    uint32_t off = block_base[blockIdx.x] + block_excl_scan((uint32_t)__popc(bits), sm, &total);
    const int64_t p0 = ((int64_t)blockIdx.x * SCAN_THREADS + threadIdx.x) * SCAN_POS_PER_THREAD;
    while (bits) { const int b = __ffs((int)bits) - 1; bits &= bits - 1; if (off < cap) out[off] = (int32_t)(p0 + b); ++off; }
}

__global__ void k_events(const int32_t *__restrict__ cand, Count nc, const uint8_t *__restrict__ ref, SegTab seg,
                         WalkParams wp, Event *__restrict__ ev, uint32_t *__restrict__ max_del)
{
    const uint32_t n_cand = count_of(nc);
    const uint32_t k = blockIdx.x * blockDim.x + threadIdx.x;
    if (k < n_cand) {
        const int64_t g = cand[k];
        const uint32_t sk = seg_of(seg, g);
        const RngKey key{wp.seed, seg.cindex[sk]};
        const int64_t p = g - seg.start[sk], l = seg.len[sk];
        const uint32_t c = ref[g];
        const U4 b1 = rng_block<false>(key, D_WALK, (uint64_t)p, 0, 0, 1);
        const U4 b2 = rng_block<false>(key, D_WALK, (uint64_t)p, 0, 0, 2);
        Event e; e.pos = (int32_t)g; e.live = 1; e.len = 1; e.base = (uint8_t)c; e.seg = sk;
        if (u_lo(b1) >= wp.indel_frac) {
            e.type = 1;
            e.base = (uint8_t)((c + (uint32_t)(uint64_t)(u_hi(b1) * 3.0 + 1)) & 3);
            e.hap = (wp.is_hap || u_lo(b2) < 0.333333) ? 3 : (u_hi(b2) < 0.5 ? 1 : 2);
        } else if (u_hi(b1) < 0.5) {
            e.type = 2;
            e.hap = (wp.is_hap || u_lo(b2) < 0.3333333) ? 3 : (u_hi(b2) < 0.5 ? 1 : 2);
            uint32_t len = 1;
            for (int64_t q = p + 1; q < l; ++q) {
                if ((int64_t)len < wp.indel_min || rng_slot<false>(key, D_WALK, (uint64_t)q, 0, 0) < wp.indel_extend) ++len; else break;
            }
            e.len = len;
            atomicMax(max_del, len);
        } else {
            e.type = 3;
            uint64_t num = 0; uint32_t kk = 0;
            do { ++num; } while (num < 0xFFFFFFFFull && ((int64_t)num < wp.indel_min || rng_slot<false>(key, D_WALK_INSLEN, (uint64_t)p, 0, kk++) < wp.indel_extend));
            e.len = (uint32_t)num;
            e.hap = (wp.is_hap || u_lo(b2) < 0.333333) ? 3 : (u_hi(b2) < 0.5 ? 1 : 2);
        }
        ev[k] = e;
    }
}

DW_DEV bool reached_by_any(const Event *ev, uint32_t k, uint32_t max_del)
{
    const int64_t pk = ev[k].pos;
    for (int64_t j = (int64_t)k - 1; j >= 0; --j) {
        const int64_t pj = ev[j].pos;
        if (pk - pj >= (int64_t)max_del) break;
        if (ev[j].type == 2 && pj + (int64_t)ev[j].len - 1 >= pk) return true;
    }
    return false;
}
__global__ void k_resolve(Event *ev, Count nc, const uint32_t *max_del_p, uint4 *flags)
{
    const uint32_t n_cand = count_of(nc);
    const uint32_t k = blockIdx.x * blockDim.x + threadIdx.x;
    if (k >= n_cand) return;
    const uint32_t max_del = *max_del_p;
    bool live = true;
    if (max_del > 1 && reached_by_any(ev, k, max_del)) {
        int64_t a = (int64_t)k - 1;
        while (a > 0 && reached_by_any(ev, (uint32_t)a, max_del)) --a;
        int64_t reach = -1;
        for (int64_t m = a; m <= (int64_t)k; ++m) {
            const bool lv = ev[m].pos > reach;
            if (lv && ev[m].type == 2) reach = (int64_t)ev[m].pos + ev[m].len - 1;
            live = lv;
        }
    }
    const Event e = ev[k];
    uint4 f;
    f.x = (live && e.type == 3 && (e.hap & 1)) ? 1u : 0u;
    f.y = (live && e.type == 3 && (e.hap & 1)) ? e.len : 0u;
    f.z = (live && e.type == 3 && (e.hap & 2)) ? 1u : 0u;
    f.w = (live && e.type == 3 && (e.hap & 2)) ? e.len : 0u;
    if (!live) f.x |= 0x80000000u;
    flags[k] = f;
}

constexpr uint32_t WALK_SEGS = 32;
static uint32_t g_walk_seg_min_rows = 16384;
void walk_debug_seg_min(uint32_t rows) { g_walk_seg_min_rows = rows ? rows : 16384; }
__global__ void k_scan4(uint4 *flags, Count nc, uint32_t *tot, uint32_t seglen, uint4 *part)
{
    const uint32_t n = count_of(nc);
    const uint32_t lo = seglen ? blockIdx.x * seglen : 0u, hi = seglen ? (lo + seglen < n ? lo + seglen : n) : n;
    constexpr uint32_t ITEMS = 8;
    __shared__ uint32_t sm[2][4][16];
    uint32_t c0 = 0, c1 = 0, c2 = 0, c3 = 0; int buf = 0;
    for (uint32_t base = lo; base < hi; base += blockDim.x * ITEMS, buf ^= 1) {
        const uint32_t i0 = base + threadIdx.x * ITEMS;
        uint4 v[ITEMS];
#pragma unroll
        for (uint32_t q = 0; q < ITEMS; ++q) v[q] = i0 + q < hi ? flags[i0 + q] : make_uint4(0, 0, 0, 0);
        uint32_t t[4] = {0, 0, 0, 0};
#pragma unroll
        for (uint32_t q = 0; q < ITEMS; ++q) {
            const uint32_t dead = v[q].x & 0x80000000u, x = v[q].x & 0x7fffffffu, y = v[q].y, z = v[q].z, w = v[q].w;
            v[q] = make_uint4(t[0] | dead, t[1], t[2], t[3]);
            t[0] += x; t[1] += y; t[2] += z; t[3] += w;
        }
        uint32_t ex[4], total[4];
        block_excl_scan_n<4>(t, sm[buf], ex, total);
#pragma unroll
        for (uint32_t q = 0; q < ITEMS; ++q)
            if (i0 + q < hi) flags[i0 + q] = make_uint4(((v[q].x & 0x7fffffffu) + ex[0] + c0) | (v[q].x & 0x80000000u), v[q].y + ex[1] + c1, v[q].z + ex[2] + c2, v[q].w + ex[3] + c3);
        c0 += total[0]; c1 += total[1]; c2 += total[2]; c3 += total[3];
    }
    if (threadIdx.x == 0) { if (seglen) part[blockIdx.x] = make_uint4(c0, c1, c2, c3); else { tot[0] = c0; tot[1] = c1; tot[2] = c2; tot[3] = c3; } }
}
__global__ void k_scan4_fix(uint4 *flags, Count nc, uint32_t *tot, uint32_t seglen, const uint4 *part)
{
    const uint32_t n = count_of(nc), i = blockIdx.x * blockDim.x + threadIdx.x, s = i / seglen;
    uint32_t a0 = 0, a1 = 0, a2 = 0, a3 = 0, t0 = 0, t1 = 0, t2 = 0, t3 = 0;
    for (uint32_t q = 0; q < WALK_SEGS; ++q) { const uint4 p = part[q]; if (q < s) { a0 += p.x; a1 += p.y; a2 += p.z; a3 += p.w; } t0 += p.x; t1 += p.y; t2 += p.z; t3 += p.w; }
    if (i == 0) { tot[0] = t0; tot[1] = t1; tot[2] = t2; tot[3] = t3; }
    if (i < n && s) { const uint4 f = flags[i]; flags[i] = make_uint4(((f.x & 0x7fffffffu) + a0) | (f.x & 0x80000000u), f.y + a1, f.z + a2, f.w + a3); }
}

__global__ void k_apply(Event *ev, Count nc, const uint4 *flags, ContigDev c, WalkParams wp)
{
    const uint32_t n_cand = count_of(nc);
    adopt_device_sizes(c);
    if (c.tot4 && (c.tot4[1] > c.cap_bases[0] || c.tot4[3] > c.cap_bases[1])) return;
    const uint32_t k = blockIdx.x * blockDim.x + threadIdx.x;
    if (k >= n_cand) return;
    const uint4 f = flags[k];
    Event e = ev[k];
    if (f.x & 0x80000000u) { ev[k].live = 0; return; }
    const int64_t p = e.pos;
    if (e.type == 1) {
        if (e.hap & 1) c.hap[0].cells[p] = T_SUB | e.base;
        if (e.hap & 2) c.hap[1].cells[p] = T_SUB | e.base;
    } else if (e.type == 2) {
        for (uint32_t q = 0; q < e.len; ++q) {
            const uint8_t v = T_DEL | c.ref[p + q];
            if (e.hap & 1) c.hap[0].cells[p + q] = v;
            if (e.hap & 2) c.hap[1].cells[p + q] = v;
        }
    } else {
        const RngKey key{wp.seed, c.seg.cindex[e.seg]};
        const uint64_t pl = (uint64_t)(p - c.seg.start[e.seg]);
        const uint32_t idx[2] = {f.x & 0x7fffffffu, f.z}, off[2] = {f.y, f.w};
        for (int h = 0; h < 2; ++h) if (e.hap & (1 << h)) {
            c.hap[h].cells[p] = T_INS | e.base;
            c.hap[h].ins_pos[idx[h]] = (int32_t)p;
            c.hap[h].ins_len[idx[h]] = e.len;
            c.hap[h].ins_off[idx[h]] = off[h];
        }
        for (uint32_t j = 0; j < e.len; ++j) {
            const uint8_t b = (uint8_t)(uint64_t)(rng_slot<false>(key, D_WALK_INSBASE, pl, 0, j) * 4.0);
            if (e.hap & 1) c.hap[0].ins_bases[off[0] + e.len - 1 - j] = b;
            if (e.hap & 2) c.hap[1].ins_bases[off[1] + e.len - 1 - j] = b;
        }
    }
}

DW_DEV void justify_ins(HapDev &h, int64_t i, int64_t lo)
{
    const uint32_t idx = ins_find(h, i);
    const uint32_t n = h.ins_len[idx];
    uint8_t *P = h.ins_bases + h.ins_off[idx];
    int64_t j = i;
    while (j > lo && (h.cells[j - 1] & TMASK) == T_NONE && P[n - 1] == (h.cells[j - 1] & 3)) {
        for (uint32_t t = n - 1; t > 0; --t) P[t] = P[t - 1];
        P[0] = h.cells[j - 1] & 3;
        h.cells[j] = h.cells[j] & 3;
        --j;
    }
    h.cells[j] = T_INS | (h.cells[j] & 3);
    h.ins_pos[idx] = (int32_t)j;
}
DW_DEV void del_swap(HapDev &h, int64_t j, int64_t dl)
{
    const uint8_t t = h.cells[j]; h.cells[j] = h.cells[j + dl]; h.cells[j + dl] = (uint8_t)((t | TMASK) ^ TMASK);
}
DW_DEV int64_t del_run(const HapDev &h, int64_t i, int64_t l)
{
    int64_t dl = 1;
    for (int64_t j = i + 1; j < l && (h.cells[j] & TMASK) == T_DEL; ++j) ++dl;
    return dl;
}
DW_DEV void justify_visit(ContigDev &c, int64_t i, int *prev_del, int64_t lo, int64_t hi)
{
    if (c.ref[i] >= 4) return;
    HapDev &h0 = c.hap[0], &h1 = c.hap[1];
    const uint8_t c1 = h0.cells[i], c2 = h1.cells[i];
    if ((c1 & TMASK) == T_NONE && (c2 & TMASK) == T_NONE) { prev_del[0] = prev_del[1] = 0; return; }
    if ((c1 & BTMASK) == (c2 & BTMASK)) {
        if ((c1 & TMASK) == T_SUB) { prev_del[0] = prev_del[1] = 0; }
        else if ((c1 & TMASK) == T_DEL) {
            if (prev_del[0] == 1 || prev_del[1] == 1) return;
            prev_del[0] = prev_del[1] = 1;
            const int64_t dl = del_run(h0, i, hi);
            if (hi <= i + dl) return;
            if (i > lo) for (int64_t j = i - 1;; --j) {
                const uint8_t a = h0.cells[j], b = h1.cells[j];
                if ((a & TMASK) != T_INS && (b & TMASK) != T_INS && (a & TMASK) != T_DEL && (b & TMASK) != T_DEL
                    && (a & 3) == (h0.cells[j + dl] & 3) && (b & 3) == (h1.cells[j + dl] & 3)) { del_swap(h0, j, dl); del_swap(h1, j, dl); }
                else break;
                if (j == lo) break;
            }
        } else { prev_del[0] = prev_del[1] = 0; justify_ins(h0, i, lo); justify_ins(h1, i, lo); }
    } else {
        if ((c1 & TMASK) == T_SUB || (c2 & TMASK) == T_SUB) { prev_del[0] = prev_del[1] = 0; }
        else if ((c1 & TMASK) == T_DEL || (c2 & TMASK) == T_DEL) {
            const int x = ((c1 & TMASK) == T_DEL) ? 0 : 1;
            if (prev_del[x] == 1) return;
            prev_del[x] = 1;
            HapDev &h = c.hap[x];
            const int64_t dl = del_run(h, i, hi);
            if (hi <= i + dl) return;
            if (i > lo) for (int64_t j = i - 1;; --j) {
                const uint8_t a = h.cells[j];
                if ((a & TMASK) == T_NONE && (a & 3) == (h.cells[j + dl] & 3)) del_swap(h, j, dl); else break;
                if (j == lo) break;
            }
        } else if ((c1 & TMASK) == T_INS) { prev_del[0] = prev_del[1] = 0; justify_ins(h0, i, lo); }
        else { prev_del[0] = prev_del[1] = 0; justify_ins(h1, i, lo); }
    }
}
__global__ void k_justify_seq(const Event *ev, Count nc, ContigDev c)
{
    const uint32_t n_cand = count_of(nc);
    adopt_device_sizes(c);
    if (blockIdx.x != 0 || threadIdx.x != 0) return;
    int prev_del[2] = {0, 0};
    int64_t last = -1; uint32_t cur = 0xFFFFFFFFu;
    for (uint32_t k = 0; k < n_cand; ++k) {
        const Event e = ev[k];
        if (!e.live) continue;
        const int64_t lo = c.seg.start[e.seg], hi = lo + c.seg.len[e.seg];
        if (e.seg != cur) { cur = e.seg; prev_del[0] = prev_del[1] = 0; last = lo - 1; }
        const int64_t p = e.pos, right = p + (e.type == 2 ? (int64_t)e.len - 1 : 0);
        if (prev_del[0] | prev_del[1])
            for (int64_t q = last + 1; q < p; ++q) if (c.ref[q] < 4) { prev_del[0] = prev_del[1] = 0; break; }
        for (int64_t i = p; i <= right; ++i) justify_visit(c, i, prev_del, lo, hi);
        last = right;
    }
}

DW_DEV int64_t reach_del(const ContigDev &c, int h, int64_t p, int64_t lo, int64_t hi)
{
    const int64_t L = del_run(c.hap[h], p, hi);
    const uint8_t *cl = c.hap[h].cells;
    int64_t j = p - 1;
    for (; j >= lo; --j) {
        const bool mutated = ((c.hap[0].cells[j] | c.hap[1].cells[j]) & TMASK) != 0;
        if (!(mutated || (p + L < hi && (cl[j] & 3) == (cl[j + L] & 3)))) break;
    }
    return j < lo ? lo : j;
}
DW_DEV int64_t reach_ins(const ContigDev &c, int h, int64_t p, int64_t lo)
{
    const uint32_t idx = ins_find(c.hap[h], p);
    const uint32_t n = c.hap[h].ins_len[idx];
    const uint8_t *P = c.hap[h].ins_bases + c.hap[h].ins_off[idx];
    int64_t j = p - 1; int64_t r = 0;
    for (; j >= lo; --j, ++r) {
        const bool mutated = ((c.hap[0].cells[j] | c.hap[1].cells[j]) & TMASK) != 0;
        const uint32_t last = r < (int64_t)n ? (uint32_t)P[n - 1 - r] : (uint32_t)(c.ref[p - 1 - (r - n)] & 3);
        if (!(mutated || last == (uint32_t)(c.ref[j] & 3))) break;
    }
    return j < lo ? lo : j;
}
__global__ void k_jreach(const Event *__restrict__ ev, Count nc, ContigDev c, int32_t *__restrict__ lo)
{
    const uint32_t n_cand = count_of(nc);
    adopt_device_sizes(c);
    const uint32_t k = blockIdx.x * blockDim.x + threadIdx.x;
    if (k >= n_cand) return;
    const Event e = ev[k];
    int64_t reach = 0x7fffffff;
    if (e.live) {
        const int64_t p = e.pos, lo = c.seg.start[e.seg], hi = lo + c.seg.len[e.seg];
        reach = p;
        if (e.type == 2) reach = reach_del(c, (e.hap & 1) ? 0 : 1, p, lo, hi);
        else if (e.type == 3) reach = reach_ins(c, (e.hap & 1) ? 0 : 1, p, lo);
        else if (e.type == 4) {
            for (int h = 0; h < 2; ++h) {
                const uint8_t t = c.hap[h].cells[p] & TMASK;
                int64_t r = p;
                if (t == T_DEL) r = reach_del(c, h, p, lo, hi); else if (t == T_INS) r = reach_ins(c, h, p, lo);
                if (r < reach) reach = r;
            }
        }
    }
    lo[k] = (int32_t)reach;
}
__global__ void k_sufmin(const int32_t *__restrict__ lo, Count nc, int32_t *__restrict__ sufmin, uint32_t seglen, int32_t *part)
{
    const uint32_t n = count_of(nc);
    const int64_t a = seglen ? (int64_t)blockIdx.x * seglen : 0, b = seglen ? (a + seglen < (int64_t)n ? a + seglen : (int64_t)n) : (int64_t)n;
    __shared__ int32_t sm[2][16];
    int32_t carry = 0x7fffffff; int buf = 0;
    const int lane = lane_id(), wave = (int)(threadIdx.x >> 6), nw = (int)(blockDim.x >> 6);
    const uint32_t nchunk = b > a ? (uint32_t)((b - a + blockDim.x - 1) / blockDim.x) : 0u;
    for (uint32_t ch = 0; ch < nchunk; ++ch, buf ^= 1) {
        const int64_t i = b - 1 - ((int64_t)ch * blockDim.x + threadIdx.x);
        int32_t v = i >= a ? lo[i] : 0x7fffffff;
#pragma unroll
        for (int d = 1; d < 64; d <<= 1) { const int32_t o = __shfl_up(v, d); if (lane >= d && o < v) v = o; }
        if (lane == 63) sm[buf][wave] = v;
        __syncthreads();
        int32_t pre = carry, all = carry;
        for (int w = 0; w < nw; ++w) { const int32_t t = sm[buf][w]; if (t < all) all = t; if (w < wave && t < pre) pre = t; }
        if (pre < v) v = pre;
        if (i >= a) sufmin[i] = v;
        carry = all;
    }
    if (seglen && threadIdx.x == 0) part[blockIdx.x] = carry;
}
__global__ void k_sufmin_fix(int32_t *__restrict__ sufmin, Count nc, uint32_t seglen, const int32_t *__restrict__ part)
{
    const uint32_t n = count_of(nc), i = blockIdx.x * blockDim.x + threadIdx.x, s = i / seglen;
    int32_t m = 0x7fffffff;
    for (uint32_t q = 0; q < WALK_SEGS; ++q) { const int32_t p = part[q]; if (q > s && p < m) m = p; }
    if (i < n && m < sufmin[i]) sufmin[i] = m;
}
__global__ void k_jbound(const Event *__restrict__ ev, Count nc, ContigDev c, const int32_t *__restrict__ sufmin, uint8_t *__restrict__ bound)
{
    const uint32_t n_cand = count_of(nc);
    adopt_device_sizes(c);
    const uint32_t k = blockIdx.x * blockDim.x + threadIdx.x;
    if (k >= n_cand) return;
    uint8_t b = 0;
    if (ev[k].live) {
        int64_t a = (int64_t)k - 1;
        while (a >= 0 && !ev[a].live) --a;
        if (a < 0 || ev[a].seg != ev[k].seg) b = 1;
        else {
            const int64_t right_a = (int64_t)ev[a].pos + (ev[a].type == 2 ? (int64_t)ev[a].len - 1 : 0);
            if ((int64_t)sufmin[k] > right_a) {
                for (int64_t q = right_a + 1; q < (int64_t)ev[k].pos; ++q) if (c.ref[q] < 4) { b = 1; break; }
            }
        }
    }
    bound[k] = b;
}
__global__ void k_jrun(const Event *__restrict__ ev, Count nc, ContigDev c, const uint8_t *__restrict__ bound)
{
    const uint32_t n_cand = count_of(nc);
    adopt_device_sizes(c);
    const uint32_t k0 = blockIdx.x * blockDim.x + threadIdx.x;
    if (k0 >= n_cand || !bound[k0]) return;
    int prev_del[2] = {0, 0};
    int64_t last = -1;
    for (uint32_t k = k0; k < n_cand; ++k) {
        const Event e = ev[k];
        if (!e.live) continue;
        if (k > k0 && bound[k]) break;
        const int64_t p = e.pos, right = p + (e.type == 2 ? (int64_t)e.len - 1 : 0);
        const int64_t lo = c.seg.start[e.seg], hi = lo + c.seg.len[e.seg];
        if (k > k0 && (prev_del[0] | prev_del[1]))
            for (int64_t q = last + 1; q < p; ++q) if (c.ref[q] < 4) { prev_del[0] = prev_del[1] = 0; break; }
        for (int64_t i = p; i <= right; ++i) justify_visit(c, i, prev_del, lo, hi);
        last = right;
    }
}

__global__ void k_apply_patches(const int32_t *__restrict__ pos, const uint16_t *__restrict__ cells, uint32_t n, uint8_t *h0, uint8_t *h1)
{
    const uint32_t k = blockIdx.x * blockDim.x + threadIdx.x;
    if (k < n) { h0[pos[k]] = (uint8_t)(cells[k] & 0xff); h1[pos[k]] = (uint8_t)(cells[k] >> 8); }
}

__global__ void k_collect_mask(const uint8_t *__restrict__ h0, const uint8_t *__restrict__ h1, int64_t l,
                               uint16_t *__restrict__ mask, uint32_t *__restrict__ block_count)
{
    __shared__ uint32_t sm[17];
    const int64_t p0 = ((int64_t)blockIdx.x * SCAN_THREADS + threadIdx.x) * SCAN_POS_PER_THREAD;
    uint32_t bits = 0;
    if (p0 < l) {
        const uint4 a = *reinterpret_cast<const uint4 *>(h0 + p0), b = *reinterpret_cast<const uint4 *>(h1 + p0);
        const uint32_t m[4] = {(a.x | b.x) & 0x30303030u, (a.y | b.y) & 0x30303030u, (a.z | b.z) & 0x30303030u, (a.w | b.w) & 0x30303030u};
#pragma unroll
        for (int q = 0; q < 16; ++q) if (((m[q >> 2] >> (8 * (q & 3))) & 0xff) && p0 + q < l) bits |= 1u << q;
    }
    mask[(int64_t)blockIdx.x * SCAN_THREADS + threadIdx.x] = (uint16_t)bits;
    uint32_t total;
    (void)block_excl_scan((uint32_t)__popc(bits), sm, &total);
    if (threadIdx.x == 0) block_count[blockIdx.x] = total;
}
__global__ void k_gather(const int32_t *__restrict__ pos, uint32_t n, const uint8_t *__restrict__ ref, const uint8_t *__restrict__ h0, const uint8_t *__restrict__ h1, uint32_t *__restrict__ cells)
{
    const uint32_t k = blockIdx.x * blockDim.x + threadIdx.x;
    if (k < n) { const int32_t p = pos[k]; cells[k] = (uint32_t)h0[p] | ((uint32_t)h1[p] << 8) | ((uint32_t)ref[p] << 16) | ((uint32_t)(p > 0 ? ref[p - 1] : 4) << 24); }
}

DW_DEV uint32_t hap_char(uint32_t code) { return code < 4u ? (0x54474341u >> (8u * code)) & 0xffu : (uint32_t)'N'; }
DW_DEV uint32_t hap_cell(const uint4 &v, int q) { const uint32_t w = (q & 8) ? ((q & 4) ? v.w : v.z) : ((q & 4) ? v.y : v.x); return (w >> (8 * (q & 3))) & 0xffu; }
DW_DEV uint32_t hap_ins_entry(const HapDev &h, int64_t g)
{
    const uint32_t idx = ins_find(h, g);
    return idx < h.n_ins && (int64_t)h.ins_pos[idx] == g ? idx : h.n_ins;
}
DW_DEV uint32_t hap_emitted(const HapDev &h, int64_t g, const uint4 &v, int nv)
{
    if (((v.x | v.y | v.z | v.w) & 0x10101010u) == 0) return (uint32_t)nv;
    uint32_t n = 0;
    for (int q = 0; q < nv; ++q) {
        const uint32_t ty = hap_cell(v, q) & TMASK;
        if (ty == T_DEL) continue;
        ++n;
        if (ty == T_INS) { const uint32_t idx = hap_ins_entry(h, g + q); if (idx < h.n_ins) n += h.ins_len[idx]; }
    }
    return n;
}
__global__ void __launch_bounds__(SCAN_THREADS) k_hap_len(HapDev h, SegTab seg, uint32_t *__restrict__ block_count)
{
    __shared__ uint32_t sm[17];
    const int64_t g0 = (int64_t)blockIdx.x * SCAN_POS_PER_BLOCK, g = g0 + (int64_t)threadIdx.x * SCAN_POS_PER_THREAD;
    const uint32_t sk = seg_of(seg, g0);
    const int64_t end = (int64_t)seg.start[sk] + seg.len[sk];
    uint32_t cnt = 0;
    if (g < end) { const uint4 v = *reinterpret_cast<const uint4 *>(h.cells + g); cnt = hap_emitted(h, g, v, end - g < 16 ? (int)(end - g) : 16); }
// ... 18 lines not shown
    const int64_t end = (int64_t)seg.start[sk] + seg.len[sk];
    uint4 v = make_uint4(0, 0, 0, 0); int nv = 0; uint32_t cnt = 0;
    if (g < end) { v = *reinterpret_cast<const uint4 *>(h.cells + g); nv = end - g < 16 ? (int)(end - g) : 16; cnt = hap_emitted(h, g, v, nv); }
    uint32_t total;
    const uint32_t off = block_excl_scan(cnt, sm, &total);
    if (total == 0) return;
    const HapRec R = rec[sk];
    const uint32_t B = block_base[blockIdx.x] - R.base0, len = R.n_bases;
    const uint64_t body = R.rec_off + R.hdr_len;
    const uint64_t body_bytes = (uint64_t)len + (width ? ((uint64_t)len + width - 1) / width : 1u);
    const bool plain = ((v.x | v.y | v.z | v.w) & 0x10101010u) == 0;
    for (uint32_t w0 = 0; w0 < total; w0 += HAP_WINDOW) {
        const uint32_t nb = total - w0 < (uint32_t)HAP_WINDOW ? total - w0 : (uint32_t)HAP_WINDOW;
        if (w0) __syncthreads();
        if (cnt && off < w0 + nb && off + cnt > w0) {
            uint32_t e = off;
            auto put = [&](uint32_t code) { if (e >= w0 && e - w0 < nb) stage[e - w0] = (uint8_t)hap_char(code); ++e; };
            for (int q = 0; q < nv; ++q) {
                const uint32_t c = hap_cell(v, q), ty = c & TMASK;
                if (ty == T_DEL) continue;
                put(c & 0xfu);
                if (!plain && ty == T_INS) {
                    const uint32_t idx = hap_ins_entry(h, g + q);
                    if (idx < h.n_ins) { const uint32_t n = h.ins_len[idx]; const uint8_t *P = h.ins_bases + h.ins_off[idx]; for (uint32_t j = 0; j < n; ++j) put(P[j]); }
                }
            }
        }
        __syncthreads();
        const uint32_t b0 = B + w0, b1 = b0 + nb;
        const uint32_t r0 = width ? b0 % width : 0u;
        const uint64_t aS = body + b0 + (width ? b0 / width : 0u);
        const uint64_t aE = body + (b1 == len ? body_bytes : (uint64_t)b1 + (width ? b1 / width : 0u));
        for (uint64_t wa = (aS & ~(uint64_t)15) + 16u * (uint64_t)threadIdx.x; wa < aE; wa += 16u * (uint64_t)SCAN_THREADS) {
            const int first = wa < aS ? (int)(aS - wa) : 0;
            const uint32_t d = (uint32_t)(wa + (uint64_t)first - aS), x = r0 + d;
            uint32_t line = 0, col = x;
            if (width) { line = x / (width + 1u); col = x - line * (width + 1u); }
            uint32_t bl = line * width + col - r0;
            uint32_t out[4] = {0, 0, 0, 0};
#pragma unroll
            for (int i = 0; i < 16; ++i) {
                if (i < first || wa + (uint64_t)i >= aE) continue;
                const bool nl = width && col == width;
                const uint32_t ch = (nl || bl >= nb) ? (uint32_t)'\n' : (uint32_t)stage[bl];
                if (nl) col = 0; else { ++col; ++bl; }
                out[i >> 2] |= ch << (8 * (i & 3));
            }
            if (first == 0 && wa + 16u <= aE) *reinterpret_cast<uint4 *>(text + wa) = make_uint4(out[0], out[1], out[2], out[3]);
            else {
#pragma unroll
                for (int i = 0; i < 16; ++i) if (i >= first && wa + (uint64_t)i < aE) text[wa + (uint64_t)i] = (uint8_t)(out[i >> 2] >> (8 * (i & 3)));
            }
        }
    }
}

void launch_hap_len(hipStream_t st, HapDev h, SegTab seg, int64_t l, uint32_t *block_count)
{
    if (l > 0) hipLaunchKernelGGL(k_hap_len, dim3(cdiv((uint64_t)l, SCAN_POS_PER_BLOCK)), dim3(SCAN_THREADS), 0, st, h, seg, block_count);
}
void launch_hap_write(hipStream_t st, HapDev h, SegTab seg, int64_t l, const uint32_t *block_base, const HapRec *rec, uint32_t n_rec, const uint8_t *pool, uint32_t width, uint8_t *text)
{
    if (n_rec) hipLaunchKernelGGL(k_hap_headers, dim3(n_rec < 4096u ? n_rec : 4096u), dim3(64), 0, st, rec, n_rec, pool, text);
    if (l > 0) hipLaunchKernelGGL(k_hap_write, dim3(cdiv((uint64_t)l, SCAN_POS_PER_BLOCK)), dim3(SCAN_THREADS), 0, st, h, seg, block_base, rec, width, text);
}
void launch_pack(hipStream_t st, const uint8_t *ascii, uint8_t *ref, uint8_t *h0, uint8_t *h1, int64_t l)
{
    const uint64_t nchunk = (uint64_t)(l + 15) >> 4;
    uint32_t nb = cdiv(nchunk, 256); if (nb > (1u << 16)) nb = 1u << 16; if (nb == 0) nb = 1;
    hipLaunchKernelGGL(k_pack, dim3(nb), dim3(256), 0, st, ascii, ref, h0, h1, l);
}
void launch_site_scan_list(hipStream_t st, const uint8_t *refview, int64_t l, SegTab seg, WalkParams wp, uint64_t *status, uint64_t *ticket, int32_t *out, uint32_t cap, uint64_t *n_out)
{
    const uint32_t nb = (uint32_t)cdiv((uint64_t)l, (uint64_t)SITE_BLOCK_POS);
    hipLaunchKernelGGL(k_site_scan_list, dim3(nb), dim3(SITE_THREADS), 0, st, refview, l, seg, wp, status, ticket, out, cap, n_out, nb);
}
uint32_t site_scan_blocks(int64_t l) { return (uint32_t)cdiv((uint64_t)l, (uint64_t)SITE_BLOCK_POS); }
uint32_t site_scan_block_positions() { return (uint32_t)SITE_BLOCK_POS; }
void launch_site_scan_slots(hipStream_t st, const uint8_t *refview, int64_t l, SegTab seg, WalkParams wp, int32_t *slots, uint32_t slot_cap, uint32_t *aux, int32_t *out, uint32_t cap, uint64_t *n_out, uint32_t *over)
{
    const uint32_t nb = site_scan_blocks(l);
    if (!nb) return;
    hipLaunchKernelGGL(k_site_scan_slots, dim3(nb), dim3(SITE_THREADS), 0, st, refview, l, seg, wp, slots, slot_cap, aux);
    hipLaunchKernelGGL(k_slot_scan, dim3(1), dim3(1024), 0, st, aux, nb, slot_cap, aux + nb, n_out, over);
    hipLaunchKernelGGL(k_slot_gather, dim3(nb), dim3(256), 0, st, slots, slot_cap, aux, aux + nb, out, cap);
}
void launch_mark_dirty(hipStream_t st, const Event *ev, Count n, const int32_t *lo, uint32_t *dirty)
{
    if (n.host) hipLaunchKernelGGL(k_mark_dirty, dim3(cdiv(n.host, 256)), dim3(256), 0, st, ev, n, lo, dirty);
}
void launch_dirty_chunks(hipStream_t st, bool restore, const uint32_t *dirty, uint32_t n_words, int64_t l_live, const uint8_t *ref, const uint8_t *refview, const uint16_t *refsumm, const uint16_t *refsumm2,
                         uint8_t *cells0, uint8_t *cells1, uint8_t *view0, uint8_t *view1, uint16_t *summ0, uint16_t *summ1, uint16_t *summ2_0, uint16_t *summ2_1)
{
    if (!n_words) return;
    bool per_chunk = (uint64_t)n_words * 32 <= (1ull << 21);
    if (const char *e = getenv("DWGSIM_HIP_DIRTY_MAP")) per_chunk = e[0] == 'c';
    const dim3 grid(cdiv((uint64_t)n_words * (per_chunk ? 32 : 1), 256));
    if (restore) { if (per_chunk) hipLaunchKernelGGL((k_dirty_chunks<true, true>), grid, dim3(256), 0, st, dirty, n_words, l_live, ref, refview, refsumm, refsumm2, cells0, cells1, view0, view1, summ0, summ1, summ2_0, summ2_1); else hipLaunchKernelGGL((k_dirty_chunks<true, false>), grid, dim3(256), 0, st, dirty, n_words, l_live, ref, refview, refsumm, refsumm2, cells0, cells1, view0, view1, summ0, summ1, summ2_0, summ2_1); }
    else { if (per_chunk) hipLaunchKernelGGL((k_dirty_chunks<false, true>), grid, dim3(256), 0, st, dirty, n_words, l_live, ref, refview, refsumm, refsumm2, cells0, cells1, view0, view1, summ0, summ1, summ2_0, summ2_1); else hipLaunchKernelGGL((k_dirty_chunks<false, false>), grid, dim3(256), 0, st, dirty, n_words, l_live, ref, refview, refsumm, refsumm2, cells0, cells1, view0, view1, summ0, summ1, summ2_0, summ2_1); }
}
void launch_scan_excl(hipStream_t st, uint32_t *data, uint32_t n, uint64_t *total_out)
{
    hipLaunchKernelGGL(k_scan_excl, dim3(1), dim3(1024), 0, st, data, n, total_out);
}
void launch_compact(hipStream_t st, const uint16_t *mask, const uint32_t *block_base, int32_t *out, int64_t l, uint32_t cap)
{
    hipLaunchKernelGGL(k_compact, dim3(cdiv((uint64_t)l, SCAN_POS_PER_BLOCK)), dim3(SCAN_THREADS), 0, st, mask, block_base, out, cap);
}
void launch_events(hipStream_t st, const int32_t *cand, Count n, const uint8_t *ref, SegTab seg, WalkParams wp, Event *ev, uint32_t *max_del)
{
    if (n.host) hipLaunchKernelGGL(k_events, dim3(cdiv(n.host, 256)), dim3(256), 0, st, cand, n, ref, seg, wp, ev, max_del);
}
void launch_resolve(hipStream_t st, Event *ev, Count n, const uint32_t *max_del, uint4 *flags, uint32_t *tot4)
{
    if (n.host) hipLaunchKernelGGL(k_resolve, dim3(cdiv(n.host, 256)), dim3(256), 0, st, ev, n, max_del, flags);
    if (n.host < g_walk_seg_min_rows) { hipLaunchKernelGGL(k_scan4, dim3(1), dim3(1024), 0, st, flags, n, tot4, 0u, (uint4 *)nullptr); return; }
    const uint32_t seglen = (n.host + WALK_SEGS - 1) / WALK_SEGS;
    hipLaunchKernelGGL(k_scan4, dim3(WALK_SEGS), dim3(1024), 0, st, flags, n, tot4, seglen, flags + n.host);
    hipLaunchKernelGGL(k_scan4_fix, dim3(cdiv(n.host, 256)), dim3(256), 0, st, flags, n, tot4, seglen, (const uint4 *)(flags + n.host));
}
void launch_apply(hipStream_t st, Event *ev, Count n, const uint4 *flags, ContigDev c, WalkParams wp)
{
    if (n.host) hipLaunchKernelGGL(k_apply, dim3(cdiv(n.host, 256)), dim3(256), 0, st, ev, n, flags, c, wp);
}
void launch_justify_seq(hipStream_t st, const Event *ev, Count n, ContigDev c)
{
    if (n.host) hipLaunchKernelGGL(k_justify_seq, dim3(1), dim3(64), 0, st, ev, n, c);
}
void launch_justify(hipStream_t st, const Event *ev, Count n, ContigDev c, int32_t *lo, int32_t *sufmin, uint8_t *bound)
{
    if (!n.host) return;
    hipLaunchKernelGGL(k_jreach, dim3(cdiv(n.host, 256)), dim3(256), 0, st, ev, n, c, lo);
    if (n.host < g_walk_seg_min_rows) hipLaunchKernelGGL(k_sufmin, dim3(1), dim3(1024), 0, st, lo, n, sufmin, 0u, (int32_t *)nullptr);
    else {
        const uint32_t seglen = (n.host + WALK_SEGS - 1) / WALK_SEGS;
        hipLaunchKernelGGL(k_sufmin, dim3(WALK_SEGS), dim3(1024), 0, st, lo, n, sufmin, seglen, sufmin + n.host);
        hipLaunchKernelGGL(k_sufmin_fix, dim3(cdiv(n.host, 256)), dim3(256), 0, st, sufmin, n, seglen, (const int32_t *)(sufmin + n.host));
    }
    hipLaunchKernelGGL(k_jbound, dim3(cdiv(n.host, 256)), dim3(256), 0, st, ev, n, c, sufmin, bound);
    hipLaunchKernelGGL(k_jrun, dim3(cdiv(n.host, 64)), dim3(64), 0, st, ev, n, c, bound);
}
__global__ void __launch_bounds__(SCAN_THREADS) k_mut_debug(const uint8_t *__restrict__ ref, const uint8_t *__restrict__ h0, const uint8_t *__restrict__ h1, int64_t l, uint64_t *verdict)
{
    const int64_t first = ((int64_t)blockIdx.x * SCAN_THREADS + threadIdx.x) * SCAN_POS_PER_THREAD;
    if (first >= l) return;
    const uint4 a = *reinterpret_cast<const uint4 *>(h0 + first), b = *reinterpret_cast<const uint4 *>(h1 + first);
    if ((((a.x | a.y | a.z | a.w) | (b.x | b.y | b.z | b.w)) & 0x30303030u) == 0) return;
    const uint4 r = *reinterpret_cast<const uint4 *>(ref + first);
    const uint32_t aw[4] = {a.x, a.y, a.z, a.w}, bw[4] = {b.x, b.y, b.z, b.w}, rw[4] = {r.x, r.y, r.z, r.w};
    for (int q = 0; q < SCAN_POS_PER_THREAD && first + q < l; ++q) {
        const uint32_t c0 = (rw[q >> 2] >> (8 * (q & 3))) & 0xffu, c1 = (aw[q >> 2] >> (8 * (q & 3))) & 0xffu, c2 = (bw[q >> 2] >> (8 * (q & 3))) & 0xffu;
        if (c0 >= 4 || ((c1 & TMASK) == T_NONE && (c2 & TMASK) == T_NONE)) continue;
        uint32_t code = 0;
        if ((c1 & BTMASK) == (c2 & BTMASK)) { if ((c1 & TMASK) == T_SUB && (c0 & 3) == (c1 & 3)) code = 1; }
        else if ((c1 & TMASK) == T_SUB || (c2 & TMASK) == T_SUB) {
            if ((c1 & 3) == (c2 & 3)) code = 2;
            else if (!((c0 & 3) == (c1 & 3) || (c0 & 3) == (c2 & 3))) code = 3;
        }
        if (code) { atomicMin((unsigned long long *)verdict, ((unsigned long long)(first + q) << 8) | code); return; }
    }
}
void launch_mut_debug(hipStream_t st, const uint8_t *ref, const uint8_t *h0, const uint8_t *h1, int64_t l, uint64_t *verdict)
{
    if (l > 0) hipLaunchKernelGGL(k_mut_debug, dim3(cdiv((uint64_t)l, SCAN_POS_PER_BLOCK)), dim3(SCAN_THREADS), 0, st, ref, h0, h1, l, verdict);
}
__global__ void __launch_bounds__(256) k_make_view(const uint8_t *__restrict__ cells0, const uint8_t *__restrict__ cells1, int64_t n_cells, int64_t l_live, uint8_t *__restrict__ view0, uint8_t *__restrict__ view1,
                                                   uint16_t *__restrict__ summ0, uint16_t *__restrict__ summ1, uint16_t *__restrict__ summ2_0, uint16_t *__restrict__ summ2_1)
{
    const uint8_t *__restrict__ cells = blockIdx.y ? cells1 : cells0;
    uint8_t *__restrict__ view = blockIdx.y ? view1 : view0;
    uint16_t *__restrict__ summ = blockIdx.y ? summ1 : summ0, *__restrict__ summ2 = blockIdx.y ? summ2_1 : summ2_0;
    const int64_t t = (int64_t)blockIdx.x * 256 + threadIdx.x, first = t * 32;
    const bool live = first < n_cells;
    uint32_t out[4] = {0, 0, 0, 0}, indel = 0, non_acgt = 0;
    if (live) {
#pragma unroll
        for (int q = 0; q < 2; ++q) {
            if (first + 16 * q >= n_cells) break;
            const uint4 v = *reinterpret_cast<const uint4 *>(cells + first + 16 * q);
            const uint32_t w[4] = {v.x, v.y, v.z, v.w};
#pragma unroll
            for (int b = 0; b < 16; ++b) {
                const uint32_t c = (w[b >> 2] >> (8 * (b & 3))) & 0xffu, ty = c & TMASK, base = c & 0xfu;
                const uint32_t nib = ty == T_NONE ? (base < 4 ? base : base == 4 ? 8u : 9u) : (ty == T_SUB && base < 4) ? 4u + base : 15u;
                const int cell = 16 * q + b;
                out[cell >> 3] |= nib << (4 * (cell & 7));
            }
#pragma unroll
            for (int k = 0; k < 4; ++k) {
                const int64_t rem = l_live - (first + 16 * q + 4 * k);
                const uint32_t lm = rem >= 4 ? 0xFFFFFFFFu : rem <= 0 ? 0u : ((1u << (8 * (int)rem)) - 1u);
                indel += (uint32_t)__popc(w[k] & lm & 0x10101010u);
                non_acgt |= w[k] & lm & 0x0C0C0C0Cu;
            }
        }
        *reinterpret_cast<uint4 *>(view + (first >> 1)) = make_uint4(out[0], out[1], out[2], out[3]);
    }
    uint32_t i1 = indel, f1 = non_acgt ? 1u : 0u;
#pragma unroll
    for (int d = 1; d < SUMM_CELLS / 32; d <<= 1) { i1 += (uint32_t)__shfl_xor((int)i1, d); f1 |= (uint32_t)__shfl_xor((int)f1, d); }
    uint32_t i2 = i1, f2 = f1;
#pragma unroll
    for (int d = SUMM_CELLS / 32; d < SUMM2_CELLS / 32; d <<= 1) { i2 += (uint32_t)__shfl_xor((int)i2, d); f2 |= (uint32_t)__shfl_xor((int)f2, d); }
    if (first < l_live) {
        if ((t & (SUMM_CELLS / 32 - 1)) == 0) summ[t / (SUMM_CELLS / 32)] = (uint16_t)(i1 | (f1 ? 0x8000u : 0u));
        if ((t & (SUMM2_CELLS / 32 - 1)) == 0) summ2[t / (SUMM2_CELLS / 32)] = (uint16_t)(i2 | (f2 ? 0x8000u : 0u));
    }
}
void launch_make_view(hipStream_t st, const uint8_t *cells0, const uint8_t *cells1, int64_t n_cells, int64_t l_live, uint8_t *view0, uint8_t *view1, uint16_t *summ0, uint16_t *summ1, uint16_t *summ2_0, uint16_t *summ2_1)
{
    if (n_cells > 0) hipLaunchKernelGGL(k_make_view, dim3(cdiv((uint64_t)n_cells, 256 * 32), 2), dim3(256), 0, st, cells0, cells1, n_cells, l_live, view0, view1, summ0, summ1, summ2_0, summ2_1);
}
void launch_apply_patches(hipStream_t st, const int32_t *pos, const uint16_t *cells, uint32_t n, uint8_t *h0, uint8_t *h1)
{
    if (n) hipLaunchKernelGGL(k_apply_patches, dim3(cdiv(n, 256)), dim3(256), 0, st, pos, cells, n, h0, h1);
}
void launch_collect_mask(hipStream_t st, const uint8_t *h0, const uint8_t *h1, int64_t l, uint16_t *mask, uint32_t *block_count)
{
    hipLaunchKernelGGL(k_collect_mask, dim3(cdiv((uint64_t)l, SCAN_POS_PER_BLOCK)), dim3(SCAN_THREADS), 0, st, h0, h1, l, mask, block_count);
}
void launch_gather(hipStream_t st, const int32_t *pos, uint32_t n, const uint8_t *ref, const uint8_t *h0, const uint8_t *h1, uint32_t *cells)
{
// ... 5 lines not shown
```

Before: 1405.

## Fold fix-up, dirty-marking and counter-zeroing kernels into neighbouring walk/sim kernels

Removes several small kernel launches and copies from the mutation walk and simulate paths. Segment fix-ups for the scan and suffix-min are applied inside k_apply and k_jbound, and dirty marking moves into k_jreach. Counter zeroing moves into k_dirty_chunks, the segment table upload and fail-rule ticket into the init kernel, and the fail-rule reduction becomes a single-pass kernel with an LDS transpose. This cuts per-iteration launch and synchronisation overhead, but adds redundant per-thread loops over segment partials and more complex cross-block ordering that needs fences.

Result: faster. 1430, median of 6 (+1.8%).

```diff
diff --git a/dwgsim_amd/csrc/dw_common.hpp b/dwgsim_amd/csrc/dw_common.hpp
--- a/dwgsim_amd/csrc/dw_common.hpp
+++ b/dwgsim_amd/csrc/dw_common.hpp
@@ -157,6 +157,9 @@
 DW_DEV void status_store(uint64_t *p, uint64_t v) { __hip_atomic_store(p, v, __ATOMIC_RELAXED, __HIP_MEMORY_SCOPE_AGENT); }
 DW_DEV uint64_t status_load(uint64_t *p) { return __hip_atomic_load(p, __ATOMIC_RELAXED, __HIP_MEMORY_SCOPE_AGENT); }
 
+DW_DEV void fence_release() { __atomic_thread_fence(__ATOMIC_RELEASE); }
+DW_DEV void fence_acquire() { __atomic_thread_fence(__ATOMIC_ACQUIRE); }
+
 #ifndef DW_LB_SLEEP
 #define DW_LB_SLEEP 2
 #endif
diff --git a/dwgsim_amd/csrc/dw_host.cpp b/dwgsim_amd/csrc/dw_host.cpp
--- a/dwgsim_amd/csrc/dw_host.cpp
+++ b/dwgsim_amd/csrc/dw_host.cpp
@@ -937,17 +937,19 @@
                      M.d_summ[0].get<uint16_t>(), M.d_summ[1].get<uint16_t>(), M.d_summ2[0].get<uint16_t>(), M.d_summ2[1].get<uint16_t>());
 }
 
-static void dirty_chunks(hipStream_t st, bool restore, const Group &g)
+static void dirty_chunks(dwgsim_hip_ctx_t *c, hipStream_t st, bool restore, const Group &g)
 {
     const GroupMem &M = g.mem;
+    static_assert(WC_RANDOM.off % 4 == 0 && WC_RANDOM.bytes % 4 == 0 && WC_RANDOM.bytes / 4 <= 256, "the opening kernel zeroes the span in 32-bit words, its first block alone");
     launch_dirty_chunks(st, restore, M.d_dirty.get<uint32_t>(), dirty_words(padded_cells(g)), g.total, M.d_ref.get(), M.d_refview.get(), M.d_refsumm.get<uint16_t>(), M.d_refsumm2.get<uint16_t>(),
-                        M.d_cells[0].get(), M.d_cells[1].get(), M.d_view[0].get(), M.d_view[1].get(), M.d_summ[0].get<uint16_t>(), M.d_summ[1].get<uint16_t>(), M.d_summ2[0].get<uint16_t>(), M.d_summ2[1].get<uint16_t>());
-}
-
-static void justify(dwgsim_hip_ctx_t *c, hipStream_t st, const Event *ev, Count n, const ContigDev &cd)
+                        M.d_cells[0].get(), M.d_cells[1].get(), M.d_view[0].get(), M.d_view[1].get(), M.d_summ[0].get<uint16_t>(), M.d_summ[1].get<uint16_t>(), M.d_summ2[0].get<uint16_t>(), M.d_summ2[1].get<uint16_t>(),
+                        reinterpret_cast<uint32_t *>(c->d_wcounters.get() + WC_RANDOM.off), (uint32_t)(WC_RANDOM.bytes / 4));
+}
+
+static void justify(dwgsim_hip_ctx_t *c, hipStream_t st, const Event *ev, Count n, const ContigDev &cd, uint32_t *dirty)
 {
     if (c->seq_justify) launch_justify_seq(st, ev, n, cd);
-    else launch_justify(st, ev, n, cd, c->w_lo.get<int32_t>(), c->w_sufmin.get<int32_t>(), c->w_bound.get<uint8_t>());
+    else launch_justify(st, ev, n, cd, c->w_lo.get<int32_t>(), c->w_sufmin.get<int32_t>(), c->w_bound.get<uint8_t>(), dirty);
 }
 
 static int64_t pack_walk_form(int attempt, bool file_driven, bool slots, int restore, bool dense)
@@ -974,7 +976,7 @@
         if (nev) HIPC(c, hipMemcpyAsync(c->w_ev.get(), c->h_pev.data(), sizeof(Event) * nev, hipMemcpyHostToDevice, st));
         launch_apply_patches(st, c->w_ppos.get<int32_t>(), c->w_pcells.get<uint16_t>(), np, M.d_cells[0].get(), M.d_cells[1].get());
         launch_mut_debug(st, M.d_ref.get(), M.d_cells[0].get(), M.d_cells[1].get(), g.total, &wc->mut_debug[0]);
-        if (nev) justify(c, st, c->w_ev.get<Event>(), Count{nullptr, nev}, group_dev(g));
+        if (nev) justify(c, st, c->w_ev.get<Event>(), Count{nullptr, nev}, group_dev(g), nullptr);
         launch_mut_debug(st, M.d_ref.get(), M.d_cells[0].get(), M.d_cells[1].get(), g.total, &wc->mut_debug[1]);
     }
     make_views(st, g);
@@ -1032,7 +1034,7 @@
     int32_t *d_cand = c->w_cand.get<int32_t>(); Event *d_ev = c->w_ev.get<Event>(); uint4 *d_flags = c->w_flags.get<uint4>();
     uint32_t *tot4 = &wc->ins[0].entries;
     const Count nc{&wc->n_cand, P.cap};
-    HIPC(c, wc_fill(c, WC_RANDOM, 0, st));
+    if (P.restore != Restore::Chunks) HIPC(c, wc_fill(c, WC_RANDOM, 0, st));
     if (P.use_slots) launch_site_scan_slots(st, M.d_refview.get(), g.total, seg, wp, c->w_slots.get<int32_t>(), P.slot_cap, c->w_slot_aux.get<uint32_t>(), d_cand, P.cap, &wc->n_cand, &wc->slot_over);
     else {
         uint64_t *d_status = c->scratch_status.get<uint64_t>();
@@ -1043,14 +1045,13 @@
     launch_resolve(st, d_ev, nc, &wc->max_del, d_flags, tot4);
     ContigDev cd = group_dev(g);
     cd.tot4 = tot4; cd.cap_bases[0] = (uint32_t)std::min<size_t>(ins_bases_cap(g, 0), 0xFFFFFFFFu); cd.cap_bases[1] = (uint32_t)std::min<size_t>(ins_bases_cap(g, 1), 0xFFFFFFFFu);
-    launch_apply(st, d_ev, nc, d_flags, cd, wp);
-    justify(c, st, d_ev, nc, cd);
+    launch_apply(st, d_ev, nc, d_flags, cd, wp, tot4);
+    justify(c, st, d_ev, nc, cd, P.dense ? nullptr : M.d_dirty.get<uint32_t>());
     if (P.dense) {
         make_views(st, g);
         g.dirty_all = true;
     } else {
-        launch_mark_dirty(st, d_ev, nc, c->w_lo.get<int32_t>(), M.d_dirty.get<uint32_t>());
-        dirty_chunks(st, false, g);
+        dirty_chunks(c, st, false, g);
         g.dirty_any = true;
     }
     HIPC(c, hipGetLastError());
@@ -1065,8 +1066,9 @@
     hipStream_t st = c->walk_stream;
     HIPC(c, hipEventRecord(g.mem.ev_walk0.get(), st));
     if (P.restore == Restore::All) { for (int h = 0; h < 2; ++h) if (const int rc = restore_pristine(c, g, h, R_ALL, st)) return rc; }
-    else if (P.restore == Restore::Chunks) dirty_chunks(st, true, g);
-    if (P.restore != Restore::None) { if (const int rc = clear_dirty(c, g, st)) return rc; g.dirty_all = g.dirty_any = false; }
+    else if (P.restore == Restore::Chunks) dirty_chunks(c, st, true, g);
+    if (P.restore == Restore::All) { if (const int rc = clear_dirty(c, g, st)) return rc; }
+    if (P.restore != Restore::None) g.dirty_all = g.dirty_any = false;
     if (const int rc = walk_launch(c, g, P)) return rc;
     HIPC(c, wc_fetch(c, g.mem, WC_RANDOM, st));
     HIPC(c, hipEventRecord(g.mem.ev_walk.get(), st));
@@ -1728,7 +1730,7 @@
     if (!f.split) P.status = 4 * sizeof(uint64_t) * nblk;
     else { P.split_state = sizeof(uint32_t) * (size_t)f.lds_words * SIM_THREADS * nblk; P.split_hand = 16 * (size_t)SIM_THREADS * nblk; P.split_agg = 16 * nblk; P.split_pre = 32 * nblk; P.split_chunk = 32 * (nblk / 1024 + 1); }
     P.meta = sizeof(uint32_t) * ((size_t)n_pairs + 8);
-    P.fail_summ = ((size_t)((n_pairs + 256ull * 64 - 1) / (256ull * 64)) * 4 + 2) * sizeof(uint64_t);
+    P.fail_summ = ((size_t)failrule_blocks(n_pairs) * 4 + 2) * sizeof(uint64_t);
     P.scratch = f.dt == 2 || (f.dt < 2 && f.nthr == SIM_THREADS_LONG);
     if (P.scratch) {
         const int cu_per_xcd = (c->n_cu >= 64 && c->n_cu % 8 == 0) ? c->n_cu / 8 : c->n_cu;
@@ -1788,7 +1790,6 @@
     if (n_pairs == 0) { if (ch.set_rand || ch.set_carry) launch_chain_set(c->stream, ch.words, rand_base, ch.set_rand, ch.carry, ch.set_carry); return DWGSIM_HIP_OK; }
     uint32_t opens = 0; for (const SimSeg &s : L.segs) opens |= s.contig_start;
     memcpy(sl.h_segs.get(), L.segs.data(), P.segs);
-    HIPC(c, hipMemcpyAsync(sl.segs.get(), sl.h_segs.get(), P.segs, hipMemcpyHostToDevice, c->stream));
     a.segs = sl.segs.get<SimSeg>(); a.n_seg = (int32_t)L.segs.size(); a.n_blocks = nblk; a.n_pairs = n_pairs; a.chain = ch.words; a.lb_shift = P.lb_shift;
     a.meta = c->meta.get<uint32_t>(); a.block_rand = c->block_rand.get<uint32_t>(); a.counters = sl.counters.dev();
     for (int t = 0; t < 3; ++t) a.out[t] = c->out[slot][t].get<uint8_t>();
@@ -1796,8 +1797,9 @@
     if (f.split) { a.split_state = c->split_state.get<uint32_t>(); a.split_hand = c->split_hand.get<uint32_t>(); a.split_agg = c->split_agg.get<uint32_t>(); a.split_pre = c->split_pre.get<uint64_t>(); a.split_chunk = c->split_chunk.get<uint64_t>(); }
     if (P.scratch) { a.flow_scratch = c->flow_scratch.get<uint32_t>(); a.flow_free = c->flow_free.get<uint64_t>(); a.flow_slots = P.flow_slots; }
     sl.group = c->handles[(size_t)L.g->first_handle].group;
+    static_assert(sizeof(SimSeg) % 4 == 0, "launch_init copies the range table in 32-bit words");
     launch_init(c->stream, sl.counters.dev(), (uint32_t)N_COUNTERS, a.status[0], f.split ? 0 : 4 * (uint64_t)nblk, a.flow_free, a.flow_free ? 256 + 8 * (uint64_t)nblk : 0,
-                ch.words, rand_base, ch.set_rand, ch.carry, ch.set_carry);
+                ch.words, rand_base, ch.set_rand, ch.carry, ch.set_carry, rerun ? nullptr : c->fail_summ.get<uint64_t>() + 4 * (size_t)failrule_blocks(n_pairs), sl.h_segs.get(), sl.segs.get(), P.segs);
     HIPC(c, hipEventRecord(sl.ev_k0, c->stream));
     c->sim_form = (int64_t)f.nthr << 20 | f.lpp << 16 | f.out << 12 | f.dt << 8 | f.wr << 4 | f.split;
     if (!launch_simulate(c->stream, a, f)) { c->err = "simulate: no k_simulate instance for this form"; return DWGSIM_HIP_ERR_FAILED; }
diff --git a/dwgsim_amd/csrc/dw_launch.hpp b/dwgsim_amd/csrc/dw_launch.hpp
--- a/dwgsim_amd/csrc/dw_launch.hpp
+++ b/dwgsim_amd/csrc/dw_launch.hpp
@@ -8,17 +8,16 @@
 uint32_t site_scan_blocks(int64_t l);
 uint32_t site_scan_block_positions();
 void launch_site_scan_slots(hipStream_t st, const uint8_t *refview, int64_t l, SegTab seg, WalkParams wp, int32_t *slots, uint32_t slot_cap, uint32_t *aux, int32_t *out, uint32_t cap, uint64_t *n_out, uint32_t *over);
-void launch_mark_dirty(hipStream_t st, const Event *ev, Count n, const int32_t *lo, uint32_t *dirty);
-void launch_dirty_chunks(hipStream_t st, bool restore, const uint32_t *dirty, uint32_t n_words, int64_t l_live, const uint8_t *ref, const uint8_t *refview, const uint16_t *refsumm, const uint16_t *refsumm2,
-                         uint8_t *cells0, uint8_t *cells1, uint8_t *view0, uint8_t *view1, uint16_t *summ0, uint16_t *summ1, uint16_t *summ2_0, uint16_t *summ2_1);
+void launch_dirty_chunks(hipStream_t st, bool restore, uint32_t *dirty, uint32_t n_words, int64_t l_live, const uint8_t *ref, const uint8_t *refview, const uint16_t *refsumm, const uint16_t *refsumm2,
+                         uint8_t *cells0, uint8_t *cells1, uint8_t *view0, uint8_t *view1, uint16_t *summ0, uint16_t *summ1, uint16_t *summ2_0, uint16_t *summ2_1, uint32_t *wc_zero, uint32_t wc_words);
 void launch_scan_excl(hipStream_t st, uint32_t *data, uint32_t n, uint64_t *total_out);
 void launch_compact(hipStream_t st, const uint16_t *mask, const uint32_t *block_base, int32_t *out, int64_t l, uint32_t cap);
 void launch_events(hipStream_t st, const int32_t *cand, Count n, const uint8_t *ref, SegTab seg, WalkParams wp, Event *ev, uint32_t *max_del);
 void walk_debug_seg_min(uint32_t rows);
 void launch_resolve(hipStream_t st, Event *ev, Count n, const uint32_t *max_del, uint4 *flags, uint32_t *tot4);
-void launch_apply(hipStream_t st, Event *ev, Count n, const uint4 *flags, ContigDev c, WalkParams wp);
+void launch_apply(hipStream_t st, Event *ev, Count n, const uint4 *flags, ContigDev c, WalkParams wp, uint32_t *tot4);
 void launch_justify_seq(hipStream_t st, const Event *ev, Count n, ContigDev c);
-void launch_justify(hipStream_t st, const Event *ev, Count n, ContigDev c, int32_t *lo, int32_t *sufmin, uint8_t *bound);
+void launch_justify(hipStream_t st, const Event *ev, Count n, ContigDev c, int32_t *lo, int32_t *sufmin, uint8_t *bound, uint32_t *dirty);
 void launch_mut_debug(hipStream_t st, const uint8_t *ref, const uint8_t *h0, const uint8_t *h1, int64_t l, uint64_t *verdict);
 void launch_make_view(hipStream_t st, const uint8_t *cells0, const uint8_t *cells1, int64_t n_cells, int64_t l_live, uint8_t *view0, uint8_t *view1, uint16_t *summ0, uint16_t *summ1, uint16_t *summ2_0, uint16_t *summ2_1);
 void launch_apply_patches(hipStream_t st, const int32_t *pos, const uint16_t *cells, uint32_t n, uint8_t *h0, uint8_t *h1);
@@ -31,7 +30,9 @@
 void launch_calibrate(hipStream_t st, const CalibArgs &a);
 void launch_failrule(hipStream_t st, const uint32_t *meta, uint64_t n_pairs, uint32_t opens_contig, uint64_t *summ, uint64_t *counters, uint64_t *chain);
 void launch_chain_set(hipStream_t st, uint64_t *chain, uint64_t rand_base, int set_rand, uint64_t carry, int set_carry);
-void launch_init(hipStream_t st, uint64_t *counters, uint32_t n_counters, uint64_t *z0, uint64_t n0, uint64_t *z1, uint64_t n1, uint64_t *chain, uint64_t rand_base, int set_rand, uint64_t carry, int set_carry);
+void launch_init(hipStream_t st, uint64_t *counters, uint32_t n_counters, uint64_t *z0, uint64_t n0, uint64_t *z1, uint64_t n1, uint64_t *chain, uint64_t rand_base, int set_rand, uint64_t carry, int set_carry,
+                 uint64_t *ticket, const void *h_segs, void *segs, size_t seg_bytes);
+uint32_t failrule_blocks(uint64_t n_pairs);
 void launch_selftest_lazy(hipStream_t st, int mode, uint32_t first, uint64_t n, double sigma, float qk, float qeps, float qlmin, int qnear1, uint64_t *out);
 uint64_t gz_chunks(uint64_t n);
 uint64_t gz_capacity(uint64_t n);
diff --git a/dwgsim_amd/csrc/dw_simulate.hip b/dwgsim_amd/csrc/dw_simulate.hip
--- a/dwgsim_amd/csrc/dw_simulate.hip
+++ b/dwgsim_amd/csrc/dw_simulate.hip
@@ -1006,64 +1006,93 @@
     }
     return x;
 }
-constexpr int FAIL_PAIRS_PER_THREAD = 64;
-__global__ void __launch_bounds__(256) k_failrule_a(const uint32_t *__restrict__ meta, uint64_t n_pairs, const uint64_t *__restrict__ counters, uint64_t *__restrict__ summ)
+constexpr int FAIL_PAIRS_PER_BLOCK = 256 * 32, FAIL_PAIRS_PER_WAVE = FAIL_PAIRS_PER_BLOCK / 4;
+DW_DEV void failrule_finish(const FailSeg &t, uint64_t *__restrict__ counters, uint64_t *__restrict__ chain)
+{
+    const uint64_t carry = chain[1];
+    const FailSeg all = failseg_join(FailSeg{carry, carry, 0, 0}, t);
+    counters[16] = t.P; counters[17] = t.S; counters[18] = t.R; counters[19] = t.bad;
+    counters[20] = (all.bad || all.P > (uint64_t)MAX_ATTEMPTS || all.S > (uint64_t)MAX_ATTEMPTS) ? 1 : 0;
+    counters[21] = all.S;
+    chain[1] = all.S;
+    counters[22] = chain[0];
+    chain[0] += counters[3];
+}
+constexpr int FAIL_PAIRS_PER_PHASE = FAIL_PAIRS_PER_WAVE / 2, FAIL_LANE_PAIRS = FAIL_PAIRS_PER_PHASE / 64, FAIL_ROW = FAIL_LANE_PAIRS + 1;
+static_assert(FAIL_LANE_PAIRS % 4 == 0 && FAIL_PAIRS_PER_PHASE % 256 == 0, "a 16-byte piece lies in one lane's row");
+__global__ void __launch_bounds__(256) k_failrule_a(const uint32_t *__restrict__ meta, uint64_t n_pairs, uint32_t opens_contig, uint64_t *__restrict__ counters, uint64_t *summ, uint64_t *__restrict__ chain)
 {
     __shared__ FailSeg seg[4];
-    if (counters[1] == 0) return;
-    const uint64_t first = ((uint64_t)blockIdx.x * 256 + threadIdx.x) * FAIL_PAIRS_PER_THREAD;
-    FailSeg s{0, 0, 0, 0};
-    for (int q4 = 0; q4 < FAIL_PAIRS_PER_THREAD && first + q4 < n_pairs; q4 += 4) {
-        const uint4 v = *reinterpret_cast<const uint4 *>(meta + first + q4);
-        const uint32_t mm[4] = {v.x, v.y, v.z, v.w};
-#pragma unroll
-        for (int u = 0; u < 4; ++u) {
-            if (first + q4 + u >= n_pairs) break;
-            const uint32_t m = mm[u];
+    __shared__ uint32_t s_last;
+    __shared__ uint32_t s_meta[4][64 * FAIL_ROW];
+    if (counters[1] == 0) {
+        if (blockIdx.x == 0 && threadIdx.x == 0) failrule_finish(FailSeg{0, 0, (counters[3] < n_pairs || opens_contig) ? 1u : 0u, 0}, counters, chain);
+        return;
+    }
+    const int lane = lane_id(), wave = (int)(threadIdx.x >> 6);
+    const uint64_t wave0 = (uint64_t)blockIdx.x * FAIL_PAIRS_PER_BLOCK + (uint64_t)wave * FAIL_PAIRS_PER_WAVE;
+    uint32_t *const row = s_meta[wave];
+    FailSeg acc{0, 0, 0, 0};
+    for (int ph = 0; ph < 2; ++ph) {
+        const uint64_t p0 = wave0 + (uint64_t)ph * FAIL_PAIRS_PER_PHASE;
+        uint4 v[FAIL_PAIRS_PER_PHASE / 256];
+#pragma unroll
+        for (int u = 0; u < FAIL_PAIRS_PER_PHASE / 256; ++u) {
+            const uint64_t first = p0 + (uint64_t)u * 256 + 4u * (uint64_t)lane;
+            v[u] = first < n_pairs ? *reinterpret_cast<const uint4 *>(meta + first) : make_uint4(0, 0, 0, 0);
+        }
+#pragma unroll
+        for (int u = 0; u < FAIL_PAIRS_PER_PHASE / 256; ++u) {
+            const int x = u * 256 + 4 * lane, at = (x / FAIL_LANE_PAIRS) * FAIL_ROW + (x % FAIL_LANE_PAIRS);
+            row[at] = v[u].x; row[at + 1] = v[u].y; row[at + 2] = v[u].z; row[at + 3] = v[u].w;
+        }
+        __syncthreads();
+        const uint64_t mine = p0 + (uint64_t)FAIL_LANE_PAIRS * (uint64_t)lane;
+        FailSeg s{0, 0, 0, 0};
+        for (int q = 0; q < FAIL_LANE_PAIRS && mine + q < n_pairs; ++q) {
+            const uint32_t m = row[lane * FAIL_ROW + q];
             if (m & 0x40000000u) s = failseg_join(s, FailSeg{0, 0, 1, 0});
             FailSeg one{m & 0x3fffffffu, 0, (m >> 31) ? 0u : 1u, 0};
             if (!one.R) one.S = one.P;
             s = failseg_join(s, one);
         }
-    }
-    s = failseg_wave_join(s, 64);
-    if ((threadIdx.x & 63) == 0) seg[threadIdx.x >> 6] = s;
+        s = failseg_wave_join(s, 64);
+        if (lane == 0) acc = failseg_join(acc, s);
+        __syncthreads();
+    }
+    if (lane == 0) seg[wave] = acc;
     __syncthreads();
     if (threadIdx.x == 0) {
         FailSeg t = seg[0];
         for (int k = 1; k < 4; ++k) t = failseg_join(t, seg[k]);
-        summ[4 * (uint64_t)blockIdx.x + 0] = t.P; summ[4 * (uint64_t)blockIdx.x + 1] = t.S;
-        summ[4 * (uint64_t)blockIdx.x + 2] = t.R; summ[4 * (uint64_t)blockIdx.x + 3] = t.bad;
-    }
-}
-__global__ void __launch_bounds__(64) k_failrule_b(const uint64_t *__restrict__ summ, uint32_t n_blocks, uint64_t n_pairs, uint32_t opens_contig, uint64_t *__restrict__ counters, uint64_t *__restrict__ chain)
-{
-    FailSeg t{0, 0, (counters[3] < n_pairs || opens_contig) ? 1u : 0u, 0};
-    if (counters[1] != 0) {
-        const uint32_t per = (n_blocks + 63) / 64, b0 = threadIdx.x * per, b1 = b0 + per < n_blocks ? b0 + per : n_blocks;
-        FailSeg x{0, 0, 0, 0};
-        for (uint32_t b = b0; b < b1; ++b) {
-            const FailSeg nx{summ[4 * (uint64_t)b], summ[4 * (uint64_t)b + 1], (uint32_t)summ[4 * (uint64_t)b + 2], (uint32_t)summ[4 * (uint64_t)b + 3]};
-            x = (b == b0) ? nx : failseg_join(x, nx);
-        }
-        t = failseg_wave_join(x, per ? (int)((n_blocks + per - 1) / per) : 0);
-    }
+        uint64_t *mine = summ + 4 * (uint64_t)blockIdx.x;
+        mine[0] = t.P; mine[1] = t.S; mine[2] = t.R; mine[3] = t.bad;
+        fence_release();
+        const unsigned long long before = atomicAdd((unsigned long long *)(summ + 4 * (uint64_t)gridDim.x), 1ull);
+        s_last = before + 1 == (unsigned long long)gridDim.x ? 1u : 0u;
+    }
+    __syncthreads();
+    if (!s_last) return;
+    fence_acquire();
+    const uint32_t n_blocks = gridDim.x, per = (n_blocks + 255) / 256, b0 = threadIdx.x * per, b1 = b0 + per < n_blocks ? b0 + per : n_blocks;
+    FailSeg x{0, 0, 0, 0};
+    for (uint32_t b = b0; b < b1; ++b) {
+        const uint64_t *sb = summ + 4 * (uint64_t)b;
+        x = failseg_join(x, FailSeg{sb[0], sb[1], (uint32_t)sb[2], (uint32_t)sb[3]});
+    }
+    x = failseg_wave_join(x, 64);
+    if (lane == 0) seg[wave] = x;
+    __syncthreads();
     if (threadIdx.x == 0) {
-        const uint64_t carry = chain[1];
-        const FailSeg all = failseg_join(FailSeg{carry, carry, 0, 0}, t);
-        counters[16] = t.P; counters[17] = t.S; counters[18] = t.R; counters[19] = t.bad;
-        counters[20] = (all.bad || all.P > (uint64_t)MAX_ATTEMPTS || all.S > (uint64_t)MAX_ATTEMPTS) ? 1 : 0;
-        counters[21] = all.S;
-        chain[1] = all.S;
-        counters[22] = chain[0];
-        chain[0] += counters[3];
-    }
-}
+        FailSeg t = seg[0];
+        for (int k = 1; k < 4; ++k) t = failseg_join(t, seg[k]);
+        failrule_finish(t, counters, chain);
+    }
+}
+uint32_t failrule_blocks(uint64_t n_pairs) { return (uint32_t)cdiv(n_pairs, (uint64_t)FAIL_PAIRS_PER_BLOCK); }
 void launch_failrule(hipStream_t st, const uint32_t *meta, uint64_t n_pairs, uint32_t opens_contig, uint64_t *summ, uint64_t *counters, uint64_t *chain)
 {
-    const uint32_t nb = cdiv(n_pairs, 256ull * FAIL_PAIRS_PER_THREAD);
-    hipLaunchKernelGGL(k_failrule_a, dim3(nb), dim3(256), 0, st, meta, n_pairs, counters, summ);
-    hipLaunchKernelGGL(k_failrule_b, dim3(1), dim3(64), 0, st, summ, nb, n_pairs, opens_contig, counters, chain);
+    hipLaunchKernelGGL(k_failrule_a, dim3(failrule_blocks(n_pairs)), dim3(256), 0, st, meta, n_pairs, opens_contig, counters, summ, chain);
 }
 __global__ void __launch_bounds__(64) k_chain_set(uint64_t *chain, uint64_t rand_base, int set_rand, uint64_t carry, int set_carry)
 {
@@ -1075,18 +1104,22 @@
 {
     hipLaunchKernelGGL(k_chain_set, dim3(1), dim3(64), 0, st, chain, rand_base, set_rand, carry, set_carry);
 }
-__global__ void __launch_bounds__(256) k_launch_init(uint64_t *counters, uint32_t n_counters, uint64_t *z0, uint64_t n0, uint64_t *z1, uint64_t n1, uint64_t *chain, uint64_t rand_base, int set_rand, uint64_t carry, int set_carry)
+__global__ void __launch_bounds__(256) k_launch_init(uint64_t *counters, uint32_t n_counters, uint64_t *z0, uint64_t n0, uint64_t *z1, uint64_t n1, uint64_t *chain, uint64_t rand_base, int set_rand, uint64_t carry, int set_carry,
+                                                     uint64_t *ticket, const uint32_t *__restrict__ h_segs, uint32_t *__restrict__ segs, uint32_t seg_words)
 {
     const uint64_t i = (uint64_t)blockIdx.x * 256 + threadIdx.x, stride = (uint64_t)gridDim.x * 256;
     if (i < n_counters) counters[i] = 0;
     for (uint64_t k = i; k < n0; k += stride) z0[k] = 0;
     for (uint64_t k = i; k < n1; k += stride) z1[k] = 0;
-    if (i == 0) { if (set_rand) chain[0] = rand_base; if (set_carry) chain[1] = carry; }
-}
-void launch_init(hipStream_t st, uint64_t *counters, uint32_t n_counters, uint64_t *z0, uint64_t n0, uint64_t *z1, uint64_t n1, uint64_t *chain, uint64_t rand_base, int set_rand, uint64_t carry, int set_carry)
+    for (uint64_t k = i; k < seg_words; k += stride) segs[k] = h_segs[k];
+    if (i == 0) { if (set_rand) chain[0] = rand_base; if (set_carry) chain[1] = carry; if (ticket) *ticket = 0; }
+}
+void launch_init(hipStream_t st, uint64_t *counters, uint32_t n_counters, uint64_t *z0, uint64_t n0, uint64_t *z1, uint64_t n1, uint64_t *chain, uint64_t rand_base, int set_rand, uint64_t carry, int set_carry,
+                 uint64_t *ticket, const void *h_segs, void *segs, size_t seg_bytes)
 {
     const uint64_t most = n0 > n1 ? n0 : n1, want = (most + 255) / 256;
-    hipLaunchKernelGGL(k_launch_init, dim3((uint32_t)(want < 1 ? 1 : want > 2048 ? 2048 : want)), dim3(256), 0, st, counters, n_counters, z0, n0, z1, n1, chain, rand_base, set_rand, carry, set_carry);
+    hipLaunchKernelGGL(k_launch_init, dim3((uint32_t)(want < 1 ? 1 : want > 2048 ? 2048 : want)), dim3(256), 0, st, counters, n_counters, z0, n0, z1, n1, chain, rand_base, set_rand, carry, set_carry,
+                       ticket, (const uint32_t *)h_segs, (uint32_t *)segs, (uint32_t)(seg_bytes / 4));
 }
 __global__ void __launch_bounds__(256) k_count_byte(const uint8_t *__restrict__ text, uint64_t n, uint32_t byte, uint64_t *out)
 {
diff --git a/dwgsim_amd/csrc/dw_walk.hip b/dwgsim_amd/csrc/dw_walk.hip
--- a/dwgsim_amd/csrc/dw_walk.hip
+++ b/dwgsim_amd/csrc/dw_walk.hip
@@ -113,85 +113,98 @@
     __syncthreads();
     if (threadIdx.x == 0) { const bool o = s_over != 0; *n_out = o ? 0ull : (uint64_t)total; if (o) { over[0] = 1u; over[1] = total; } }
 }
+constexpr uint32_t SLOT_FOLD_MAX = 4096;
 __global__ void __launch_bounds__(256) k_slot_gather(const int32_t *__restrict__ slots, uint32_t slot_cap, const uint32_t *__restrict__ slot_cnt, const uint32_t *__restrict__ slot_base,
-                                                     int32_t *__restrict__ out, uint32_t cap)
-{
-    const uint32_t t = blockIdx.x, base = slot_base[t];
+                                                     int32_t *__restrict__ out, uint32_t cap, uint64_t *n_out, uint32_t *over)
+{
+    __shared__ uint32_t sm[17];
+    __shared__ uint32_t s_over;
+    const uint32_t t = blockIdx.x;
+    uint32_t base;
+    if (slot_base) base = slot_base[t];
+    else {
+        if (threadIdx.x == 0) s_over = 0;
+        uint32_t sum = 0; bool big = false;
+        for (uint32_t q = threadIdx.x; q < t; q += 256u) { const uint32_t c = slot_cnt[q]; sum += c; big |= c > slot_cap; }
+        uint32_t total;
+        (void)block_excl_scan(sum, sm, &total);
+        base = total;
+        if (t + 1 == gridDim.x) {
+            if (big) atomicOr(&s_over, 1u);
+            __syncthreads();
+            if (threadIdx.x == 0) { const uint32_t all = base + slot_cnt[t]; const bool o = s_over != 0 || slot_cnt[t] > slot_cap; *n_out = o ? 0ull : (uint64_t)all; if (o) { over[0] = 1u; over[1] = all; } }
+        }
+    }
     uint32_t n = slot_cnt[t]; if (n > slot_cap) n = slot_cap;
     for (uint32_t k = threadIdx.x; k < n; k += 256u) if (base + k < cap) out[base + k] = slots[(size_t)t * slot_cap + k];
 }
 
-__global__ void k_mark_dirty(const Event *__restrict__ ev, Count nc, const int32_t *__restrict__ lo, uint32_t *__restrict__ dirty)
-{
-    const uint32_t n = count_of(nc), k = blockIdx.x * blockDim.x + threadIdx.x;
-    if (k >= n) return;
-    const Event e = ev[k];
-    if (!e.live) return;
+DW_DEV void mark_dirty(const Event &e, int32_t lo, uint32_t *__restrict__ dirty)
+{
     const int64_t right = (int64_t)e.pos + (e.type == 2 ? (int64_t)e.len - 1 : 0);
-    const int64_t a = (int64_t)(lo[k] < e.pos ? lo[k] : e.pos) >> 6, b = right >> 6;
+    const int64_t a = (int64_t)(lo < e.pos ? lo : e.pos) >> 6, b = right >> 6;
     for (int64_t q = a; q <= b; ++q) atomicOr(&dirty[q >> 5], 1u << (q & 31));
 }
+DW_DEV uint32_t view_nibble(uint32_t c) { const uint32_t ty = c & TMASK, base = c & 0xfu; return ty == T_NONE ? (base < 4 ? base : base == 4 ? 8u : 9u) : (ty == T_SUB && base < 4) ? 4u + base : 15u; }
 template <bool RESTORE, bool PER_CHUNK>
-__global__ void __launch_bounds__(256) k_dirty_chunks(const uint32_t *__restrict__ dirty, uint32_t n_words, int64_t l_live, const uint8_t *__restrict__ ref, const uint8_t *__restrict__ refview,
+__global__ void __launch_bounds__(256) k_dirty_chunks(uint32_t *dirty, uint32_t n_words, int64_t l_live, const uint8_t *__restrict__ ref, const uint8_t *__restrict__ refview,
                                                       const uint16_t *__restrict__ refsumm, const uint16_t *__restrict__ refsumm2,
                                                       uint8_t *__restrict__ cells0, uint8_t *__restrict__ cells1, uint8_t *__restrict__ view0, uint8_t *__restrict__ view1,
-                                                      uint16_t *__restrict__ summ0, uint16_t *__restrict__ summ1, uint16_t *__restrict__ summ2_0, uint16_t *__restrict__ summ2_1)
+                                                      uint16_t *__restrict__ summ0, uint16_t *__restrict__ summ1, uint16_t *__restrict__ summ2_0, uint16_t *__restrict__ summ2_1,
+                                                      uint32_t *__restrict__ wc_zero, uint32_t wc_words)
 {
     const uint64_t gid = (uint64_t)blockIdx.x * 256u + threadIdx.x;
+    if (RESTORE && gid < wc_words) wc_zero[gid] = 0u;
     const uint32_t w = PER_CHUNK ? (uint32_t)(gid >> 5) : (uint32_t)gid;
     const bool in = w < n_words;
     const uint32_t touched = in ? dirty[w] : 0u;
     if (PER_CHUNK) { if (!__ballot(touched != 0u)) return; }
     else if (!touched) return;
-    uint32_t bits = PER_CHUNK ? ((touched >> (gid & 31u)) & 1u) << (gid & 31u) : touched;
-    uint32_t fine[2] = {0u, 0u};
-    const bool mine = bits != 0u;
-    while (bits) {
-        const int q = __ffs((int)bits) - 1; bits &= bits - 1;
-        const int64_t ch = (int64_t)w * 32 + q, first = ch * SUMM_CELLS;
-        if (RESTORE) {
-#pragma unroll
-            for (int k = 0; k < SUMM_CELLS / 16; ++k) { const uint4 v = *reinterpret_cast<const uint4 *>(ref + first + 16 * k); *reinterpret_cast<uint4 *>(cells0 + first + 16 * k) = v; *reinterpret_cast<uint4 *>(cells1 + first + 16 * k) = v; }
-#pragma unroll
-            for (int k = 0; k < SUMM_CELLS / 32; ++k) { const uint4 v = *reinterpret_cast<const uint4 *>(refview + (first >> 1) + 16 * k); *reinterpret_cast<uint4 *>(view0 + (first >> 1) + 16 * k) = v; *reinterpret_cast<uint4 *>(view1 + (first >> 1) + 16 * k) = v; }
-            const uint16_t sv = refsumm[ch]; summ0[ch] = sv; summ1[ch] = sv;
-        } else {
-#pragma unroll
-            for (int h = 0; h < 2; ++h) {
-                const uint8_t *cells = h ? cells1 : cells0; uint8_t *view = h ? view1 : view0;
-                uint32_t indel = 0, non_acgt = 0;
-#pragma unroll
-                for (int half = 0; half < SUMM_CELLS / 32; ++half) {
-                    uint32_t out[4] = {0, 0, 0, 0};
-#pragma unroll
-                    for (int qq = 0; qq < 2; ++qq) {
-                        const int64_t at = first + 32 * half + 16 * qq;
-                        const uint4 v = *reinterpret_cast<const uint4 *>(cells + at);
-                        const uint32_t wd[4] = {v.x, v.y, v.z, v.w};
-#pragma unroll
-                        for (int b = 0; b < 16; ++b) {
-                            const uint32_t c = (wd[b >> 2] >> (8 * (b & 3))) & 0xffu, ty = c & TMASK, base = c & 0xfu;
-                            const uint32_t nib = ty == T_NONE ? (base < 4 ? base : base == 4 ? 8u : 9u) : (ty == T_SUB && base < 4) ? 4u + base : 15u;
-                            const int cell = 16 * qq + b;
-                            out[cell >> 3] |= nib << (4 * (cell & 7));
+    if (RESTORE && touched && (!PER_CHUNK || (gid & 31u) == 0u)) dirty[w] = 0u;
+    static_assert(SUMM_CELLS == 64 && SUMM2_CELLS / SUMM_CELLS == 16, "a chunk = sixteen lanes x four cells; a coarse summary = the sixteen lanes of half a bitmap word");
+    if (!PER_CHUNK) {
+        uint32_t bits = touched;
+        while (bits) {
+            const int q = __ffs((int)bits) - 1; bits &= bits - 1;
+            const int64_t ch = (int64_t)w * 32 + q, first = ch * SUMM_CELLS;
+            if (RESTORE) {
+#pragma unroll
+                for (int k = 0; k < SUMM_CELLS / 16; ++k) { const uint4 v = *reinterpret_cast<const uint4 *>(ref + first + 16 * k); *reinterpret_cast<uint4 *>(cells0 + first + 16 * k) = v; *reinterpret_cast<uint4 *>(cells1 + first + 16 * k) = v; }
+#pragma unroll
+                for (int k = 0; k < SUMM_CELLS / 32; ++k) { const uint4 v = *reinterpret_cast<const uint4 *>(refview + (first >> 1) + 16 * k); *reinterpret_cast<uint4 *>(view0 + (first >> 1) + 16 * k) = v; *reinterpret_cast<uint4 *>(view1 + (first >> 1) + 16 * k) = v; }
+                const uint16_t sv = refsumm[ch]; summ0[ch] = sv; summ1[ch] = sv;
+            } else {
+#pragma unroll
+                for (int h = 0; h < 2; ++h) {
+                    const uint8_t *cells = h ? cells1 : cells0; uint8_t *view = h ? view1 : view0;
+                    uint32_t indel = 0, non_acgt = 0;
+#pragma unroll
+                    for (int half = 0; half < SUMM_CELLS / 32; ++half) {
+                        uint32_t out[4] = {0, 0, 0, 0};
+#pragma unroll
+                        for (int qq = 0; qq < 2; ++qq) {
+                            const int64_t at = first + 32 * half + 16 * qq;
+                            const uint4 v = *reinterpret_cast<const uint4 *>(cells + at);
+                            const uint32_t wd[4] = {v.x, v.y, v.z, v.w};
+#pragma unroll
+                            for (int b = 0; b < 16; ++b) {
+                                const int cell = 16 * qq + b;
+                                out[cell >> 3] |= view_nibble((wd[b >> 2] >> (8 * (b & 3))) & 0xffu) << (4 * (cell & 7));
+                            }
+#pragma unroll
+                            for (int k = 0; k < 4; ++k) {
+                                const int64_t rem = l_live - (at + 4 * k);
+                                const uint32_t lm = rem >= 4 ? 0xFFFFFFFFu : rem <= 0 ? 0u : ((1u << (8 * (int)rem)) - 1u);
+                                indel += (uint32_t)__popc(wd[k] & lm & 0x10101010u);
+                                non_acgt |= wd[k] & lm & 0x0C0C0C0Cu;
+                            }
                         }
-#pragma unroll
-                        for (int k = 0; k < 4; ++k) {
-                            const int64_t rem = l_live - (at + 4 * k);
-                            const uint32_t lm = rem >= 4 ? 0xFFFFFFFFu : rem <= 0 ? 0u : ((1u << (8 * (int)rem)) - 1u);
-                            indel += (uint32_t)__popc(wd[k] & lm & 0x10101010u);
-                            non_acgt |= wd[k] & lm & 0x0C0C0C0Cu;
-                        }
+                        *reinterpret_cast<uint4 *>(view + ((first + 32 * half) >> 1)) = make_uint4(out[0], out[1], out[2], out[3]);
                     }
-                    *reinterpret_cast<uint4 *>(view + ((first + 32 * half) >> 1)) = make_uint4(out[0], out[1], out[2], out[3]);
+                    (h ? summ1 : summ0)[ch] = (uint16_t)(indel | (non_acgt ? 0x8000u : 0u));
                 }
-                fine[h] = indel | (non_acgt ? 0x8000u : 0u);
-                (h ? summ1 : summ0)[ch] = (uint16_t)fine[h];
-            }
-        }
-    }
-    static_assert(SUMM2_CELLS / SUMM_CELLS == 16, "a coarse summary = the sixteen lanes of half a bitmap word");
-    if (!PER_CHUNK) {
+            }
+        }
 #pragma unroll
         for (int half = 0; half < 2; ++half) {
             if (!((touched >> (16 * half)) & 0xFFFFu)) continue;
@@ -210,6 +223,53 @@
         }
         return;
     }
+    const int lane = (int)(gid & 63u), grp = lane >> 4, j = lane & 15;
+    const uint64_t m = (uint64_t)(uint32_t)__shfl((int)touched, 0) | ((uint64_t)(uint32_t)__shfl((int)touched, 32) << 32);
+    const int64_t ch0 = (int64_t)(gid >> 6) * 64;
+    const int n_dirty = __popcll(m);
+    const bool mine = (m >> lane) & 1ull;
+    const int rank = __popcll(m & ((1ull << lane) - 1ull));
+    uint32_t fine[2] = {0u, 0u};
+    uint64_t left = m;
+    for (int r = 0; 4 * r < n_dirty; ++r) {
+        uint64_t mm = left;
+        for (int k = 0; k < grp; ++k) mm &= mm - 1;
+        const bool work = mm != 0;
+        const int64_t ch = ch0 + (work ? __ffsll((unsigned long long)mm) - 1 : 0), first = ch * SUMM_CELLS + 4 * j;
+        for (int k = 0; k < 4; ++k) left &= left - 1;
+        uint32_t f[2] = {0u, 0u};
+        if (RESTORE) {
+            if (work) {
+                const uint32_t v = *reinterpret_cast<const uint32_t *>(ref + first);
+                *reinterpret_cast<uint32_t *>(cells0 + first) = v; *reinterpret_cast<uint32_t *>(cells1 + first) = v;
+                const uint16_t vv = *reinterpret_cast<const uint16_t *>(refview + (first >> 1));
+                *reinterpret_cast<uint16_t *>(view0 + (first >> 1)) = vv; *reinterpret_cast<uint16_t *>(view1 + (first >> 1)) = vv;
+                if (j == 0) { const uint16_t sv = refsumm[ch]; summ0[ch] = sv; summ1[ch] = sv; }
+            }
+        } else {
+#pragma unroll
+            for (int h = 0; h < 2; ++h) {
+                uint32_t indel = 0, non_acgt = 0;
+                if (work) {
+                    const uint32_t wd = *reinterpret_cast<const uint32_t *>((h ? cells1 : cells0) + first);
+                    uint32_t out = 0;
+#pragma unroll
+                    for (int b = 0; b < 4; ++b) out |= view_nibble((wd >> (8 * b)) & 0xffu) << (4 * b);
+                    *reinterpret_cast<uint16_t *>((h ? view1 : view0) + (first >> 1)) = (uint16_t)out;
+                    const int64_t rem = l_live - first;
+                    const uint32_t lm = rem >= 4 ? 0xFFFFFFFFu : rem <= 0 ? 0u : ((1u << (8 * (int)rem)) - 1u);
+                    indel = (uint32_t)__popc(wd & lm & 0x10101010u);
+                    non_acgt = wd & lm & 0x0C0C0C0Cu;
+                }
+#pragma unroll
+                for (int d = 1; d < 16; d <<= 1) { indel += (uint32_t)__shfl_xor((int)indel, d); non_acgt |= (uint32_t)__shfl_xor((int)non_acgt, d); }
+                f[h] = indel | (non_acgt ? 0x8000u : 0u);
+                if (work && j == 0) (h ? summ1 : summ0)[ch] = (uint16_t)f[h];
+                const uint32_t got = (uint32_t)__shfl((int)f[h], (rank & 3) * 16);
+                if (mine && (rank >> 2) == r) fine[h] = got;
+            }
+        }
+    }
     const int q = (int)(gid & 31u);
     const int64_t ch = (int64_t)w * 32 + q;
     const int64_t s2 = (int64_t)w * 2 + (q >> 4);
@@ -222,7 +282,7 @@
             if (live2 && ch * SUMM_CELLS < l_live) v = mine ? fine[h] : (uint32_t)(h ? summ1 : summ0)[ch];
             uint32_t cnt = v & 0x7fffu, fl = v & 0x8000u;
 #pragma unroll
-            for (int m = 1; m < 16; m <<= 1) { cnt += (uint32_t)__shfl_xor((int)cnt, m); fl |= (uint32_t)__shfl_xor((int)fl, m); }
+            for (int mk = 1; mk < 16; mk <<= 1) { cnt += (uint32_t)__shfl_xor((int)cnt, mk); fl |= (uint32_t)__shfl_xor((int)fl, mk); }
             if (live2 && (q & 15) == 0) (h ? summ2_1 : summ2_0)[s2] = (uint16_t)(cnt | fl);
         }
     }
@@ -359,23 +419,24 @@
     }
     if (threadIdx.x == 0) { if (seglen) part[blockIdx.x] = make_uint4(c0, c1, c2, c3); else { tot[0] = c0; tot[1] = c1; tot[2] = c2; tot[3] = c3; } }
 }
-__global__ void k_scan4_fix(uint4 *flags, Count nc, uint32_t *tot, uint32_t seglen, const uint4 *part)
-{
-    const uint32_t n = count_of(nc), i = blockIdx.x * blockDim.x + threadIdx.x, s = i / seglen;
-    uint32_t a0 = 0, a1 = 0, a2 = 0, a3 = 0, t0 = 0, t1 = 0, t2 = 0, t3 = 0;
-    for (uint32_t q = 0; q < WALK_SEGS; ++q) { const uint4 p = part[q]; if (q < s) { a0 += p.x; a1 += p.y; a2 += p.z; a3 += p.w; } t0 += p.x; t1 += p.y; t2 += p.z; t3 += p.w; }
-    if (i == 0) { tot[0] = t0; tot[1] = t1; tot[2] = t2; tot[3] = t3; }
-    if (i < n && s) { const uint4 f = flags[i]; flags[i] = make_uint4(((f.x & 0x7fffffffu) + a0) | (f.x & 0x80000000u), f.y + a1, f.z + a2, f.w + a3); }
-}
-
-__global__ void k_apply(Event *ev, Count nc, const uint4 *flags, ContigDev c, WalkParams wp)
+
+__global__ void k_apply(Event *ev, Count nc, const uint4 *flags, ContigDev c, WalkParams wp, uint32_t seglen, const uint4 *__restrict__ part, uint32_t *tot_out)
 {
     const uint32_t n_cand = count_of(nc);
-    adopt_device_sizes(c);
-    if (c.tot4 && (c.tot4[1] > c.cap_bases[0] || c.tot4[3] > c.cap_bases[1])) return;
     const uint32_t k = blockIdx.x * blockDim.x + threadIdx.x;
+    uint32_t a0 = 0, a1 = 0, a2 = 0, a3 = 0;
+    if (seglen) {
+        const uint32_t s = k / seglen;
+        uint32_t t0 = 0, t1 = 0, t2 = 0, t3 = 0;
+        for (uint32_t q = 0; q < WALK_SEGS; ++q) { const uint4 p = part[q]; if (q < s) { a0 += p.x; a1 += p.y; a2 += p.z; a3 += p.w; } t0 += p.x; t1 += p.y; t2 += p.z; t3 += p.w; }
+        if (k == 0) { tot_out[0] = t0; tot_out[1] = t1; tot_out[2] = t2; tot_out[3] = t3; }
+        if (t1 > c.cap_bases[0] || t3 > c.cap_bases[1]) return;
+    } else {
+        if (c.tot4 && (c.tot4[1] > c.cap_bases[0] || c.tot4[3] > c.cap_bases[1])) return;
+    }
     if (k >= n_cand) return;
-    const uint4 f = flags[k];
+    uint4 f = flags[k];
+    f = make_uint4(((f.x & 0x7fffffffu) + a0) | (f.x & 0x80000000u), f.y + a1, f.z + a2, f.w + a3);
     Event e = ev[k];
     if (f.x & 0x80000000u) { ev[k].live = 0; return; }
     const int64_t p = e.pos;
@@ -514,7 +575,7 @@
     }
     return j < lo ? lo : j;
 }
-__global__ void k_jreach(const Event *__restrict__ ev, Count nc, ContigDev c, int32_t *__restrict__ lo)
+__global__ void k_jreach(const Event *__restrict__ ev, Count nc, ContigDev c, int32_t *__restrict__ lo, uint32_t *__restrict__ dirty)
 {
     const uint32_t n_cand = count_of(nc);
     adopt_device_sizes(c);
@@ -537,6 +598,7 @@
         }
     }
     lo[k] = (int32_t)reach;
+    if (dirty && e.live) mark_dirty(e, (int32_t)reach, dirty);
 }
 __global__ void k_sufmin(const int32_t *__restrict__ lo, Count nc, int32_t *__restrict__ sufmin, uint32_t seglen, int32_t *part)
 {
@@ -561,14 +623,7 @@
     }
     if (seglen && threadIdx.x == 0) part[blockIdx.x] = carry;
 }
-__global__ void k_sufmin_fix(int32_t *__restrict__ sufmin, Count nc, uint32_t seglen, const int32_t *__restrict__ part)
-{
-    const uint32_t n = count_of(nc), i = blockIdx.x * blockDim.x + threadIdx.x, s = i / seglen;
-    int32_t m = 0x7fffffff;
-    for (uint32_t q = 0; q < WALK_SEGS; ++q) { const int32_t p = part[q]; if (q > s && p < m) m = p; }
-    if (i < n && m < sufmin[i]) sufmin[i] = m;
-}
-__global__ void k_jbound(const Event *__restrict__ ev, Count nc, ContigDev c, const int32_t *__restrict__ sufmin, uint8_t *__restrict__ bound)
+__global__ void k_jbound(const Event *__restrict__ ev, Count nc, ContigDev c, const int32_t *__restrict__ sufmin, uint8_t *__restrict__ bound, uint32_t seglen, const int32_t *__restrict__ part)
 {
     const uint32_t n_cand = count_of(nc);
     adopt_device_sizes(c);
@@ -581,7 +636,9 @@
         if (a < 0 || ev[a].seg != ev[k].seg) b = 1;
         else {
             const int64_t right_a = (int64_t)ev[a].pos + (ev[a].type == 2 ? (int64_t)ev[a].len - 1 : 0);
-            if ((int64_t)sufmin[k] > right_a) {
+            int32_t sm = sufmin[k];
+            if (seglen) { const uint32_t s = k / seglen; for (uint32_t q = s + 1; q < WALK_SEGS; ++q) { const int32_t p = part[q]; if (p < sm) sm = p; } }
+            if ((int64_t)sm > right_a) {
                 for (int64_t q = right_a + 1; q < (int64_t)ev[k].pos; ++q) if (c.ref[q] < 4) { b = 1; break; }
             }
         }
@@ -766,22 +823,21 @@
     const uint32_t nb = site_scan_blocks(l);
     if (!nb) return;
     hipLaunchKernelGGL(k_site_scan_slots, dim3(nb), dim3(SITE_THREADS), 0, st, refview, l, seg, wp, slots, slot_cap, aux);
+    if (nb <= SLOT_FOLD_MAX) { hipLaunchKernelGGL(k_slot_gather, dim3(nb), dim3(256), 0, st, slots, slot_cap, aux, (const uint32_t *)nullptr, out, cap, n_out, over); return; }
     hipLaunchKernelGGL(k_slot_scan, dim3(1), dim3(1024), 0, st, aux, nb, slot_cap, aux + nb, n_out, over);
-    hipLaunchKernelGGL(k_slot_gather, dim3(nb), dim3(256), 0, st, slots, slot_cap, aux, aux + nb, out, cap);
-}
-void launch_mark_dirty(hipStream_t st, const Event *ev, Count n, const int32_t *lo, uint32_t *dirty)
-{
-    if (n.host) hipLaunchKernelGGL(k_mark_dirty, dim3(cdiv(n.host, 256)), dim3(256), 0, st, ev, n, lo, dirty);
-}
-void launch_dirty_chunks(hipStream_t st, bool restore, const uint32_t *dirty, uint32_t n_words, int64_t l_live, const uint8_t *ref, const uint8_t *refview, const uint16_t *refsumm, const uint16_t *refsumm2,
-                         uint8_t *cells0, uint8_t *cells1, uint8_t *view0, uint8_t *view1, uint16_t *summ0, uint16_t *summ1, uint16_t *summ2_0, uint16_t *summ2_1)
+    hipLaunchKernelGGL(k_slot_gather, dim3(nb), dim3(256), 0, st, slots, slot_cap, aux, aux + nb, out, cap, n_out, over);
+}
+void launch_dirty_chunks(hipStream_t st, bool restore, uint32_t *dirty, uint32_t n_words, int64_t l_live, const uint8_t *ref, const uint8_t *refview, const uint16_t *refsumm, const uint16_t *refsumm2,
+                         uint8_t *cells0, uint8_t *cells1, uint8_t *view0, uint8_t *view1, uint16_t *summ0, uint16_t *summ1, uint16_t *summ2_0, uint16_t *summ2_1, uint32_t *wc_zero, uint32_t wc_words)
 {
     if (!n_words) return;
     bool per_chunk = (uint64_t)n_words * 32 <= (1ull << 21);
     if (const char *e = getenv("DWGSIM_HIP_DIRTY_MAP")) per_chunk = e[0] == 'c';
     const dim3 grid(cdiv((uint64_t)n_words * (per_chunk ? 32 : 1), 256));
-    if (restore) { if (per_chunk) hipLaunchKernelGGL((k_dirty_chunks<true, true>), grid, dim3(256), 0, st, dirty, n_words, l_live, ref, refview, refsumm, refsumm2, cells0, cells1, view0, view1, summ0, summ1, summ2_0, summ2_1); else hipLaunchKernelGGL((k_dirty_chunks<true, false>), grid, dim3(256), 0, st, dirty, n_words, l_live, ref, refview, refsumm, refsumm2, cells0, cells1, view0, view1, summ0, summ1, summ2_0, summ2_1); }
-    else { if (per_chunk) hipLaunchKernelGGL((k_dirty_chunks<false, true>), grid, dim3(256), 0, st, dirty, n_words, l_live, ref, refview, refsumm, refsumm2, cells0, cells1, view0, view1, summ0, summ1, summ2_0, summ2_1); else hipLaunchKernelGGL((k_dirty_chunks<false, false>), grid, dim3(256), 0, st, dirty, n_words, l_live, ref, refview, refsumm, refsumm2, cells0, cells1, view0, view1, summ0, summ1, summ2_0, summ2_1); }
+#define DW_DIRTY_ARGS dirty, n_words, l_live, ref, refview, refsumm, refsumm2, cells0, cells1, view0, view1, summ0, summ1, summ2_0, summ2_1, wc_zero, wc_words
+    if (restore) { if (per_chunk) hipLaunchKernelGGL((k_dirty_chunks<true, true>), grid, dim3(256), 0, st, DW_DIRTY_ARGS); else hipLaunchKernelGGL((k_dirty_chunks<true, false>), grid, dim3(256), 0, st, DW_DIRTY_ARGS); }
+    else { if (per_chunk) hipLaunchKernelGGL((k_dirty_chunks<false, true>), grid, dim3(256), 0, st, DW_DIRTY_ARGS); else hipLaunchKernelGGL((k_dirty_chunks<false, false>), grid, dim3(256), 0, st, DW_DIRTY_ARGS); }
+#undef DW_DIRTY_ARGS
 }
 void launch_scan_excl(hipStream_t st, uint32_t *data, uint32_t n, uint64_t *total_out)
 {
@@ -798,30 +854,27 @@
 void launch_resolve(hipStream_t st, Event *ev, Count n, const uint32_t *max_del, uint4 *flags, uint32_t *tot4)
 {
     if (n.host) hipLaunchKernelGGL(k_resolve, dim3(cdiv(n.host, 256)), dim3(256), 0, st, ev, n, max_del, flags);
-    if (n.host < g_walk_seg_min_rows) { hipLaunchKernelGGL(k_scan4, dim3(1), dim3(1024), 0, st, flags, n, tot4, 0u, (uint4 *)nullptr); return; }
+    if (!n.host || n.host < g_walk_seg_min_rows) { hipLaunchKernelGGL(k_scan4, dim3(1), dim3(1024), 0, st, flags, n, tot4, 0u, (uint4 *)nullptr); return; }
     const uint32_t seglen = (n.host + WALK_SEGS - 1) / WALK_SEGS;
     hipLaunchKernelGGL(k_scan4, dim3(WALK_SEGS), dim3(1024), 0, st, flags, n, tot4, seglen, flags + n.host);
-    hipLaunchKernelGGL(k_scan4_fix, dim3(cdiv(n.host, 256)), dim3(256), 0, st, flags, n, tot4, seglen, (const uint4 *)(flags + n.host));
-}
-void launch_apply(hipStream_t st, Event *ev, Count n, const uint4 *flags, ContigDev c, WalkParams wp)
-{
-    if (n.host) hipLaunchKernelGGL(k_apply, dim3(cdiv(n.host, 256)), dim3(256), 0, st, ev, n, flags, c, wp);
+}
+void launch_apply(hipStream_t st, Event *ev, Count n, const uint4 *flags, ContigDev c, WalkParams wp, uint32_t *tot4)
+{
+    if (!n.host) return;
+    const uint32_t seglen = n.host < g_walk_seg_min_rows ? 0u : (n.host + WALK_SEGS - 1) / WALK_SEGS;
+    hipLaunchKernelGGL(k_apply, dim3(cdiv(n.host, 256)), dim3(256), 0, st, ev, n, flags, c, wp, seglen, flags + n.host, tot4);
 }
 void launch_justify_seq(hipStream_t st, const Event *ev, Count n, ContigDev c)
 {
     if (n.host) hipLaunchKernelGGL(k_justify_seq, dim3(1), dim3(64), 0, st, ev, n, c);
 }
-void launch_justify(hipStream_t st, const Event *ev, Count n, ContigDev c, int32_t *lo, int32_t *sufmin, uint8_t *bound)
+void launch_justify(hipStream_t st, const Event *ev, Count n, ContigDev c, int32_t *lo, int32_t *sufmin, uint8_t *bound, uint32_t *dirty)
 {
     if (!n.host) return;
-    hipLaunchKernelGGL(k_jreach, dim3(cdiv(n.host, 256)), dim3(256), 0, st, ev, n, c, lo);
-    if (n.host < g_walk_seg_min_rows) hipLaunchKernelGGL(k_sufmin, dim3(1), dim3(1024), 0, st, lo, n, sufmin, 0u, (int32_t *)nullptr);
-    else {
-        const uint32_t seglen = (n.host + WALK_SEGS - 1) / WALK_SEGS;
-        hipLaunchKernelGGL(k_sufmin, dim3(WALK_SEGS), dim3(1024), 0, st, lo, n, sufmin, seglen, sufmin + n.host);
-        hipLaunchKernelGGL(k_sufmin_fix, dim3(cdiv(n.host, 256)), dim3(256), 0, st, sufmin, n, seglen, (const int32_t *)(sufmin + n.host));
-    }
-    hipLaunchKernelGGL(k_jbound, dim3(cdiv(n.host, 256)), dim3(256), 0, st, ev, n, c, sufmin, bound);
+    hipLaunchKernelGGL(k_jreach, dim3(cdiv(n.host, 256)), dim3(256), 0, st, ev, n, c, lo, dirty);
+    const uint32_t seglen = n.host < g_walk_seg_min_rows ? 0u : (n.host + WALK_SEGS - 1) / WALK_SEGS;
+    hipLaunchKernelGGL(k_sufmin, dim3(seglen ? WALK_SEGS : 1u), dim3(1024), 0, st, lo, n, sufmin, seglen, seglen ? sufmin + n.host : (int32_t *)nullptr);
+    hipLaunchKernelGGL(k_jbound, dim3(cdiv(n.host, 256)), dim3(256), 0, st, ev, n, c, sufmin, bound, seglen, (const int32_t *)(sufmin + n.host));
     hipLaunchKernelGGL(k_jrun, dim3(cdiv(n.host, 64)), dim3(64), 0, st, ev, n, c, bound);
 }
 __global__ void __launch_bounds__(SCAN_THREADS) k_mut_debug(const uint8_t *__restrict__ ref, const uint8_t *__restrict__ h0, const uint8_t *__restrict__ h1, int64_t l, uint64_t *verdict)
```
